# nh13/DWGSIM

Measured on AMD Instinct MI355X. Metric: M read-pairs/sec (2x150 bp PE), higher is better.
Workload: dtype u8

## Files before the change

### dwgsim_amd/csrc/dw_host.cpp

```cpp
#include <hip/hip_runtime.h>
#include <math.h>
#include <stdio.h>
#include <stdlib.h>
#include <string.h>
#include <limits.h>
#include <ctype.h>
#include <stdarg.h>
#include <stdint.h>
#include <sys/mman.h>
#include <mutex>
#include <thread>
#include <string>
#include <vector>
#include <algorithm>
#include <array>
#include <stddef.h>
#include <type_traits>
#include "../../include/dwgsim_hip.h"
#include "dw_kernels.hpp"
#include "dw_launch.hpp"
#include "dw_mutin.hpp"
#include "dw_mem.hpp"

using namespace dw;

namespace {

struct HostIns { std::vector<int32_t> pos; std::vector<uint32_t> len, off; std::vector<uint8_t> bases; };

struct Member {
    std::string name;
    int64_t l = 0, l_place = 0;
    uint32_t contig_index = 0;
    int32_t start = 0;
    int32_t reg_off = 0, n_reg = 0;
    uint32_t name_off = 0; int32_t name_fixed_len = 0;
    ResolvedContig rc;
};

struct GroupMem {
    DevMem d_ref, d_cells[2], d_view[2];
    DevMem d_ins_pos[2], d_ins_len[2], d_ins_off[2], d_ins_bases[2];
    DevMem d_names, d_reg, d_seg;
    std::vector<uint8_t> h_names; std::vector<int32_t> h_reg, h_seg;
    DevMem d_summ[2], d_summ2[2];
    DevMem d_refview, d_refsumm, d_refsumm2, d_dirty;
    DevEvent ev_walk, ev_walk0;
    DevMem d_hap_text[2], d_hap_rec, d_hap_pool;
    HostMem h_wc;
};

struct WalkCounters {
    uint64_t unused0[7];
    uint64_t n_cand;
    uint32_t max_del;
    struct { uint32_t entries, bases; } ins[2];
    uint32_t unused1;
    uint32_t slot_over;
    uint32_t n_cand_true;
    uint64_t mut_debug[2];
    uint64_t n_listed;
    uint64_t unused2;
};
static_assert(std::is_standard_layout<WalkCounters>::value && sizeof(WalkCounters) == 16 * 8, "the walk's counter block is 16 u64 words");
static_assert(offsetof(WalkCounters, n_cand) == 7 * 8 && offsetof(WalkCounters, max_del) == 8 * 8 && offsetof(WalkCounters, ins) == 8 * 8 + 4 && offsetof(WalkCounters, slot_over) == 8 * 8 + 6 * 4 &&
              offsetof(WalkCounters, n_cand_true) == 8 * 8 + 7 * 4 && offsetof(WalkCounters, mut_debug) == 12 * 8 && offsetof(WalkCounters, n_listed) == 14 * 8, "every counter at the word the kernels were given before the block had a type");
struct WcSpan { size_t off, bytes; };
#define WC_SPAN(first, last) WcSpan{offsetof(WalkCounters, first), offsetof(WalkCounters, last) + sizeof(WalkCounters::last) - offsetof(WalkCounters, first)}
constexpr WcSpan WC_RANDOM = WC_SPAN(n_cand, n_cand_true), WC_FILE = WC_SPAN(mut_debug, mut_debug), WC_LISTED = WC_SPAN(n_listed, n_listed);

struct Group {
    bool alive = false, mutated = false, walk_pending = false;
    int first_handle = -1;
    std::vector<Member> m;
    int64_t total = 0;
    GroupMem mem;
    uint32_t n_ins[2] = {0, 0}, n_ins_bases[2] = {0, 0};
    int fixed_max = 0;
    uint32_t n_cand = 0;
    bool dirty_any = false, dirty_all = false;
    int walk_attempt = 0; uint32_t walk_cap = 0; size_t walk_cap_bases = 0; bool walk_reset = false;
    uint32_t n_patch = 0, n_patch_ev = 0;
    bool list_valid = false; std::vector<int32_t> pos; std::vector<uint32_t> cells; HostIns ins[2];
    struct HapText { bool valid = false; int width = 0; uint64_t bytes = 0; std::vector<uint64_t> off, len; std::vector<int64_t> bases; } hap_text[2];
};

struct HandleRef { int group = -1, k = 0; };

constexpr int N_COUNTERS = 32;

struct Counters {
    DevMem d; HostMem h;
    uint64_t *dev() const { return d.get<uint64_t>(); }
    uint64_t *host() const { return h.get<uint64_t>(); }
};

struct Slot {
    Counters counters;
    hipEvent_t ev_k0 = nullptr, ev_k1 = nullptr, ev_end = nullptr, ev_done = nullptr, ev_fetched = nullptr;
    bool pending = false, empty = true, fetch_in_flight = false;
    int group = -1;
    uint64_t n_pairs = 0, out_bytes[3] = {0, 0, 0}, gz_bytes[3] = {0, 0, 0};
    DevMem gz_out[3], gz_status, segs;
    HostMem h_segs;
    std::vector<dwgsim_hip_range_t> ranges;
    DevMem d_rerun_chain;
    int cap_mult = 1;
};

}

struct dwgsim_hip_ctx {
    dwgsim_hip_params_t prm;
    std::string read_prefix;
    std::vector<uint8_t> flow;
    DevMem d_flow;
    int device = 0;
    hipStream_t stream = nullptr;
    hipStream_t copy_stream = nullptr;
    hipStream_t walk_stream = nullptr;
    hipStream_t count_stream = nullptr;
    std::string err;
    double e_by[2] = {0, 0};
    DevMem d_thr[2];
    DevMem d_thr32[2]; int e_full = 0;
    DevMem d_qbase[2]; int32_t qb_words = 1;
    DevMem d_rand_fixed; int32_t rand_fixed_len = 0;
    std::vector<Group> groups;
    std::vector<GroupMem> pool;
    std::vector<HandleRef> handles;
    DevMem meta, fail_summ, block_rand, status_all, out[DWGSIM_HIP_SLOTS][3], split_state, split_hand, split_agg, split_pre, split_chunk;
    DevMem w_slots, w_slot_aux;
    int site_slots = -1; int64_t site_slot_cap = -1;
    DevMem scratch_mask, scratch_cnt, scratch_status, w_cand, w_ev, w_flags, w_lo, w_sufmin, w_bound, w_ppos, w_pcells, up_ascii, l_pos, l_cells, place_segs, place_rand, place_list, place_aux;
    HostMem h_up; hipEvent_t ev_up = nullptr; bool up_in_flight = false;
    HostMem h_place_segs, h_range_rand;
    std::vector<int32_t> h_ppos; std::vector<uint16_t> h_pcells; std::vector<Event> h_pev;
    bool seq_justify = false, dense_view = false;
    MutInput mutin; bool has_mutin = false;
    Regions regions; bool has_regions = false;
    DevMem flow_scratch, flow_free;
    Counters counters;
    DevMem d_wcounters;
    Counters pcounters;
    Slot slot[DWGSIM_HIP_SLOTS];
    DevMem d_chain;
    int chain_contig = -1; uint64_t chain_next_ii = 0;
    bool has_carry_override = false; uint64_t carry_override = 0;
    int flow_cap_forced = 0;
    int flow_cap_mult = 1;
    int ion_lds = -1;
    int n_cu = 0; int flow_slots = 0;
    int64_t walk_cap = -1; bool phases = false; int writer = -1, force_threads = 0; int64_t place_cap = -1; uint64_t place_open = 0; double walk_us = 0, count_us = 0; int split = -1;
    int64_t sim_form = 0;
    int64_t walk_form = 0;
    hipEvent_t ev_cnt0 = nullptr, ev_cnt1 = nullptr;
    bool gzip_on = false; DevMem d_crc_table, d_crc_shift;
    HostMem h_stage;
    hipStream_t hap_stream = nullptr;
    DevEvent hap_ev[6]; double hap_len_us = 0, hap_write_us = 0, hap_copy_us = 0; bool hap_yardstick = false;
    int hap_cur[2] = {-1, -1};
    std::string txt, vcf;
};

namespace {

#define HIPC(ctx, call) do { hipError_t e_ = (call); if (e_ != hipSuccess) { char b_[512]; snprintf(b_, sizeof b_, "HIP error %s at %s:%d (%s)", hipGetErrorString(e_), __FILE__, __LINE__, #call); (ctx)->err = b_; return DWGSIM_HIP_ERR_DEVICE; } } while (0)

hipError_t dev_malloc(dwgsim_hip_ctx *c, void **p, size_t bytes)
{
    hipError_t e = DevKind::alloc(p, bytes);
    if (e == hipSuccess || c->pool.empty()) return e;
    (void)hipGetLastError();
    hipStreamSynchronize(c->walk_stream);
    c->pool.clear();
    return DevKind::alloc(p, bytes);
}

hipError_t reserve(dwgsim_hip_ctx *c, DevMem &b, size_t need, size_t want)
{
    return b.reserve(need, want, [c](void **p, size_t n) { return dev_malloc(c, p, n); });
}

int ensure(dwgsim_hip_ctx *c, DevMem &b, size_t bytes)
{
    HIPC(c, reserve(c, b, bytes, bytes + bytes / 8 + 4096));
    return 0;
}

int upload(dwgsim_hip_ctx *c, DevMem &b, const void *src, size_t n)
{
    HIPC(c, reserve(c, b, n, n));
    const hipError_t e = hipMemcpy(b.get(), src, n, hipMemcpyHostToDevice);
    if (e != hipSuccess) b.reset();
    HIPC(c, e);
    return 0;
}

template <class T> int upload_table(dwgsim_hip_ctx_t *c, DevMem &d, const std::vector<T> &h, size_t slack)
{
    HIPC(c, reserve(c, d, sizeof(T) * h.size(), sizeof(T) * (h.size() + slack)));
    HIPC(c, hipMemcpyAsync(d.get(), h.data(), sizeof(T) * h.size(), hipMemcpyHostToDevice, c->walk_stream));
    return 0;
}

uint8_t nt4(int ch)
{
    switch (ch) { case 'A': case 'a': return 0; case 'C': case 'c': return 1; case 'G': case 'g': return 2; case 'T': case 't': return 3; case '-': return 5; default: return 4; }
}

void lazy_quality_params(double sigma, float *k, float *eps, float *lmin, int32_t *near1_zero)
{
    const double two_ln2 = 2.0 * log(2.0);
    double lm = 0.98 * (0.45 / sigma) * (0.45 / sigma) / two_ln2;
    if (!(lm < 0x1p-4)) lm = 0x1p-4;
    *near1_zero = lm >= 0x1p-10 ? 1 : 0;
    if (lm < 0x1p-10) lm = 0x1p-10;
    *lmin = (float)lm;
    lm = (double)*lmin * (1.0 - 0x1p-20);
    *k = (float)(sqrt(two_ln2) * sigma);
    *eps = (float)(1.5 * sigma * (3.4e-7 / sqrt(lm) + 7.2e-6) + 0x1p-18);
}

WalkParams walk_params(const dwgsim_hip_ctx *c)
{
    WalkParams w; w.mut_rate = c->prm.mut_rate; w.indel_frac = c->prm.indel_frac; w.indel_extend = c->prm.indel_extend;
    w.indel_min = c->prm.indel_min; w.is_hap = c->prm.is_hap; w.seed = (uint32_t)c->prm.seed;
    w.mut_thr = !(c->prm.mut_rate > 0) ? 0 : c->prm.mut_rate >= 1.0 ? 0x100000000ull : (uint64_t)ceil(c->prm.mut_rate * 4294967296.0);
    flow_gap_params(w.mut_thr, &w.gap_r, &w.gap_s);
    w.lg = reinterpret_cast<const uint32_t *>(c->d_flow.get() + 64);
    return w;
}

size_t padded_cells(const Group &g) { return (size_t)g.total + CELL_PAD; }

size_t view_bytes(size_t padded) { return padded / 2; }
size_t summ_bytes(size_t padded) { return sizeof(uint16_t) * (padded / SUMM_CELLS); }
size_t summ2_bytes(size_t padded) { return sizeof(uint16_t) * (padded / SUMM2_CELLS); }
uint32_t dirty_words(size_t padded) { return (uint32_t)((padded + 32 * SUMM_CELLS - 1) / (32 * SUMM_CELLS)); }
size_t dirty_bytes(size_t padded) { return sizeof(uint32_t) * ((size_t)dirty_words(padded) + 2); }

enum : unsigned { R_CELLS = 1, R_VIEW = 2, R_SUMM = 4, R_SUMM2 = 8, R_ALL = 15 };
int restore_pristine(dwgsim_hip_ctx *c, const Group &g, int h, unsigned what, hipStream_t st)
{
    const GroupMem &M = g.mem;
    const size_t padded = padded_cells(g);
    if (what & R_CELLS) HIPC(c, hipMemcpyAsync(M.d_cells[h].get(), M.d_ref.get(), padded, hipMemcpyDeviceToDevice, st));
    if (what & R_VIEW) HIPC(c, hipMemcpyAsync(M.d_view[h].get(), M.d_refview.get(), view_bytes(padded), hipMemcpyDeviceToDevice, st));
    if (what & R_SUMM) HIPC(c, hipMemcpyAsync(M.d_summ[h].get(), M.d_refsumm.get(), summ_bytes(padded), hipMemcpyDeviceToDevice, st));
    if (what & R_SUMM2) HIPC(c, hipMemcpyAsync(M.d_summ2[h].get(), M.d_refsumm2.get(), summ2_bytes(padded), hipMemcpyDeviceToDevice, st));
    return 0;
}

int clear_dirty(dwgsim_hip_ctx *c, const Group &g, hipStream_t st)
{
    HIPC(c, hipMemsetAsync(g.mem.d_dirty.get(), 0, dirty_bytes(padded_cells(g)), st));
    return 0;
}

hipError_t wc_fill(dwgsim_hip_ctx *c, WcSpan s, int byte, hipStream_t st) { return hipMemsetAsync(c->d_wcounters.get() + s.off, byte, s.bytes, st); }
hipError_t wc_fetch(dwgsim_hip_ctx *c, const GroupMem &M, WcSpan s, hipStream_t st) { return hipMemcpyAsync(M.h_wc.get() + s.off, c->d_wcounters.get() + s.off, s.bytes, hipMemcpyDeviceToHost, st); }

struct InsTable { void *dev, *host; size_t bytes; };
std::array<InsTable, 4> ins_tables(const GroupMem &M, int h, HostIns &t)
{
    return {{{M.d_ins_pos[h].get(), t.pos.data(), sizeof(int32_t) * t.pos.size()}, {M.d_ins_len[h].get(), t.len.data(), sizeof(uint32_t) * t.len.size()},
             {M.d_ins_off[h].get(), t.off.data(), sizeof(uint32_t) * t.off.size()}, {M.d_ins_bases[h].get(), t.bases.data(), t.bases.size()}}};
}

SegTab seg_tab(const Group &g)
{
    const int n = (int)g.m.size();
    const int32_t *seg = g.mem.d_seg.get<int32_t>();
    SegTab t; t.start = seg; t.len = seg + (n + 1); t.cindex = reinterpret_cast<const uint32_t *>(seg + (2 * n + 1)); t.n = n;
    return t;
}

void fill_haps(const Group &g, HapDev (&hap)[2])
{
    const GroupMem &M = g.mem;
    for (int h = 0; h < 2; ++h) {
        hap[h].cells = M.d_cells[h].get(); hap[h].view = M.d_view[h].get(); hap[h].ins_pos = M.d_ins_pos[h].get<int32_t>(); hap[h].ins_len = M.d_ins_len[h].get<uint32_t>();
        hap[h].ins_off = M.d_ins_off[h].get<uint32_t>(); hap[h].ins_bases = M.d_ins_bases[h].get(); hap[h].n_ins = g.n_ins[h]; hap[h].pos_off = 0;
    }
}

ContigDev group_dev(const Group &g)
{
    ContigDev d;
    fill_haps(g, d.hap);
    d.ref = g.mem.d_ref.get(); d.l = g.total; d.seg = seg_tab(g);
    d.tot4 = nullptr; d.cap_bases[0] = d.cap_bases[1] = 0;
    return d;
}

size_t ins_bases_cap(const Group &g, int h) { const size_t cap = g.mem.d_ins_bases[h].cap(); return cap ? cap - 16 : 0; }

Group *get_group(dwgsim_hip_ctx_t *c, int contig, int *k = nullptr)
{
    if (!c) return nullptr;
    if (contig < 0 || (size_t)contig >= c->handles.size() || c->handles[(size_t)contig].group < 0) { c->err = "unknown contig handle"; return nullptr; }
    const HandleRef r = c->handles[(size_t)contig];
    Group &g = c->groups[(size_t)r.group];
    if (!g.alive) { c->err = "unknown contig handle"; return nullptr; }
    if (k) *k = r.k;
    return &g;
// ... 1155 lines not shown
    if (bytes) *bytes = T.len[(size_t)km];
    if (bases) *bases = T.bases[(size_t)km];
    return DWGSIM_HIP_OK;
}

int dwgsim_hip_haplotype_fetch(dwgsim_hip_ctx_t *c, int hap, uint64_t offset, void *host_dst, size_t n)
{
    if (!c) return DWGSIM_HIP_ERR_ARG;
    if (hap < 0 || hap > 1 || (!host_dst && n)) { c->err = "bad haplotype_fetch arguments"; return DWGSIM_HIP_ERR_ARG; }
    const int gid = c->hap_cur[hap];
    if (gid < 0 || !c->groups[(size_t)gid].alive || !c->groups[(size_t)gid].hap_text[hap].valid) { c->err = "haplotype_fetch: dwgsim_hip_haplotype_fasta must run first"; return DWGSIM_HIP_ERR_STATE; }
    const Group &g = c->groups[(size_t)gid];
    const uint64_t total = g.hap_text[hap].bytes;
    if (offset > total || (uint64_t)n > total - offset) { c->err = "haplotype_fetch: past the end of the text"; return DWGSIM_HIP_ERR_ARG; }
    if (n == 0) return DWGSIM_HIP_OK;
    HIPC(c, hipSetDevice(c->device));
    if (!c->hap_stream) HIPC(c, hipStreamCreate(&c->hap_stream));
    const uint8_t *src = g.mem.d_hap_text[hap].get<uint8_t>() + offset;
    if (is_page_locked(host_dst)) {
        HIPC(c, hipMemcpyAsync(host_dst, src, n, hipMemcpyDeviceToHost, c->hap_stream));
        HIPC(c, hipStreamSynchronize(c->hap_stream));
        return DWGSIM_HIP_OK;
    }
    const size_t CH = (size_t)16 << 20;
    HIPC(c, c->h_stage.reserve(2 * CH, 2 * CH));
    uint8_t *stage[2] = {c->h_stage.get<uint8_t>(), c->h_stage.get<uint8_t>() + CH};
    size_t done = 0; int b = 0;
    size_t cur = n < CH ? n : CH;
    HIPC(c, hipMemcpyAsync(stage[0], src, cur, hipMemcpyDeviceToHost, c->hap_stream));
    while (done < n) {
        HIPC(c, hipStreamSynchronize(c->hap_stream));
        const size_t next_off = done + cur, next = next_off < n ? ((n - next_off) < CH ? (n - next_off) : CH) : 0;
        if (next) HIPC(c, hipMemcpyAsync(stage[b ^ 1], src + next_off, next, hipMemcpyDeviceToHost, c->hap_stream));
        memcpy((uint8_t *)host_dst + done, stage[b], cur);
        done += cur; cur = next; b ^= 1;
    }
    return DWGSIM_HIP_OK;
}

namespace {
struct Launch { SimForm f; SimArgs a; Group *g = nullptr; std::vector<SimSeg> segs; uint64_t n_pairs = 0; uint32_t nblk = 0; int fixed_max = 0; };
struct SimPlan {
    size_t cap[3];
    int32_t lb_shift; bool too_many;
    size_t block_rand, status, meta, fail_summ, split_state, split_hand, split_agg, split_pre, split_chunk;
    bool scratch; int32_t flow_slots; size_t flow_scratch, flow_free;
    size_t segs, gz_chunks[3], gz_cap[3], gz_status;
};
struct ChainSet { uint64_t *words; int set_rand, set_carry; uint64_t carry; };
}

static int build_ranges(dwgsim_hip_ctx_t *c, const dwgsim_hip_range_t *r, int n, uint64_t ppb, Launch &L)
{
    if (!r || n < 1) { c->err = "bad range arguments"; return DWGSIM_HIP_ERR_ARG; }
    Group *g = nullptr;
    uint64_t pairs = 0, blocks = 0; int fmax = 0;
    std::vector<SimSeg> &segs = L.segs;
    segs.clear();
    for (int q = 0; q < n; ++q) {
        int k = 0;
        Group *gq = get_group(c, r[q].contig, &k);
        if (!gq) return DWGSIM_HIP_ERR_ARG;
        if (g && gq != g) { c->err = "the ranges of one call must belong to contigs that were added together (dwgsim_hip_add_contigs)"; return DWGSIM_HIP_ERR_ARG; }
        g = gq;
        if (r[q].n_pairs == 0) continue;
        const Member &m = g->m[(size_t)k];
        if (c->has_regions && m.n_reg == 0 && c->prm.rand_read < 1.0) { c->err = "dwgsim-hip: this contig has no target region (-x): the reference's placement loop would not terminate\n"; return DWGSIM_HIP_ERR_ARG; }
        SimSeg s; memset(&s, 0, sizeof s);
        s.first_block = (uint32_t)blocks; s.contig_index = m.contig_index; s.start = m.start; s.l = (int32_t)m.l;
        s.first_ii = r[q].first_ii; s.n_pairs = r[q].n_pairs; s.pair_off = pairs; s.l_place = m.l_place;
        s.reg_off = m.reg_off; s.n_reg = m.n_reg; s.name_off = m.name_off; s.name_fixed_len = m.name_fixed_len;
        s.contig_start = r[q].first_ii == 0 ? 1u : 0u;
        segs.push_back(s);
        pairs += r[q].n_pairs; blocks += (r[q].n_pairs + ppb - 1) / ppb;
        if (m.name_fixed_len > fmax) fmax = m.name_fixed_len;
        if (blocks > 0x7fffffffull) { c->err = "too many pairs in one call"; return DWGSIM_HIP_ERR_ARG; }
    }
    if (!g->mutated || g->walk_pending) { c->err = "mutate_contig must run first"; return DWGSIM_HIP_ERR_STATE; }
    L.g = g; L.n_pairs = pairs; L.nblk = (uint32_t)blocks; L.fixed_max = fmax;
    return DWGSIM_HIP_OK;
}

static int sim_form(dwgsim_hip_ctx_t *c, SimForm &f)
{
    const dwgsim_hip_params_t &p = c->prm;
    const size_t qb = (size_t)c->qb_words;
    const int lmax = p.length[0] > p.length[1] ? p.length[0] : p.length[1];
    f = SimForm();
    f.lpp = p.length[1] > 0 ? 2 : 1;
    f.out = (p.reads_output_type != 2 ? 1 : 0) | (p.reads_output_type != 1 ? 2 : 0);
    f.dt = p.data_type;
    f.nthr = SIM_THREADS;
    f.cap = lmax; f.lds_words = (lmax + 7) / 8;
    bool fifo = true;
    if (p.data_type == 0) {
        const int cap_fifo = 5, cap_reg = (p.reads_output_type == 0) ? 4 : 5;
        const int b_fifo = sim_blocks_per_cu(sim_lds_bytes((size_t)f.lds_words, SIM_THREADS, qb, true), cap_fifo), b_reg = sim_blocks_per_cu(sim_lds_bytes((size_t)f.lds_words, SIM_THREADS, qb, false), cap_reg);
        if (b_fifo < b_reg && !(p.reads_output_type == 0 && b_fifo >= 3)) fifo = false;
        if (c->writer >= 0) fifo = c->writer != 0;
    }
    const size_t need = sim_lds_bytes((size_t)f.lds_words, SIM_THREADS, qb, fifo);
    if (p.data_type != 2 && (need > SIM_LDS_BUDGET || ((sim_blocks_per_cu(need, 8) < 2 || c->force_threads == SIM_THREADS_LONG) && c->force_threads != SIM_THREADS))) {
        f.nthr = SIM_THREADS_LONG; fifo = true;
        if (sim_lds_bytes(0, SIM_THREADS_LONG, qb, true) > SIM_LDS_BUDGET) {
            char b[160]; snprintf(b, sizeof b, "dwgsim-hip: reads longer than %d bases are not supported for -c 0 / -c 1\n", (int)((SIM_LDS_BUDGET - SIM_THREADS_LONG * SIM_FIFO_BYTES) / 2 - 16));
            c->err = b; return DWGSIM_HIP_ERR_UNSUP;
        }
    }
    if (p.data_type == 2) {
        f.cap = std::max(flow_base_capacity(c), lmax) * c->flow_cap_mult;
        f.lds_words = (f.cap + 15) / 16; f.cap = 16 * f.lds_words;
        f.stack_words = std::min(FLOW_STACK_WORDS * c->flow_cap_mult, FLOW_STACK_WORDS_MAX);
        const size_t per_lane = (size_t)(f.lds_words + f.stack_words);
        const size_t need256 = sim_lds_bytes(per_lane, SIM_THREADS, qb, true), need64 = sim_lds_bytes(per_lane, ION_THREADS_SMALL, qb, true);
        int mode = c->ion_lds;
        if (mode < 0) mode = (need256 <= SIM_LDS_BUDGET && sim_blocks_per_cu(need256, 8) >= 2) ? 1 : (need64 <= SIM_LDS_BUDGET && sim_blocks_per_cu(need64, 32) >= 4) ? 2 : 0;
        if ((mode == 1 && need256 > SIM_LDS_BUDGET) || (mode == 2 && need64 > SIM_LDS_BUDGET)) mode = 0;
        f.dt = mode != 0 ? 3 : 2; f.nthr = mode == 2 ? ION_THREADS_SMALL : SIM_THREADS;
    }
    const bool split_wins = lmax <= 50;
    f.split = (p.data_type == 0 && f.nthr == SIM_THREADS && (c->split < 0 ? split_wins : c->split != 0)) ? 1 : 0;
    if (f.dt == 3 && f.nthr == SIM_THREADS && f.cap < 32768 && c->split != 0) f.split = 1;
    if (f.split && c->writer < 0) fifo = true;
    const size_t stage = f.dt == 3 ? (size_t)(f.lds_words + f.stack_words) : f.dt == 2 ? (size_t)f.stack_words : f.nthr != SIM_THREADS ? 0 : (size_t)f.lds_words;
    if (f.split) { f.wr = fifo ? 2 : 0; f.lds = sim_lds_bytes(stage, (size_t)f.nthr, 0, false); f.lds_b = sim_lds_bytes(0, (size_t)f.nthr, qb, fifo, SIM_FIFO_BYTES_WIDE); }
    else { f.wr = fifo ? 1 : 0; f.lds = sim_lds_bytes(stage, (size_t)f.nthr, qb, fifo); }
    return 0;
}

static void fill_sim_args(const dwgsim_hip_ctx_t *c, const Group &g, const SimForm &f, SimArgs &a)
{
    const dwgsim_hip_params_t &p = c->prm;
    memset(&a, 0, sizeof a);
    a.p.std_dev = p.std_dev; a.p.mut_freq = p.mut_freq; a.p.rand_read = p.rand_read; a.p.quality_std = p.quality_std;
    a.p.dist = p.dist; a.p.is_inner = p.is_inner; a.p.len[0] = p.length[0]; a.p.len[1] = p.length[1]; a.p.max_n = p.max_n;
    a.p.strandedness = p.strandedness; a.p.read_one_strand = p.read_one_strand; a.p.amplicons = p.amplicons;
    a.p.fixed_quality = p.fixed_quality; a.p.data_type = p.data_type;
    a.p.has_bfast = p.reads_output_type != 1; a.p.has_bwa = p.reads_output_type != 2;
    a.p.seed = (uint32_t)p.seed;
    lazy_quality_params(p.quality_std, &a.p.q_k, &a.p.q_eps, &a.p.q_lmin, &a.p.q_near1);
    fill_haps(g, a.hap);
    a.chain = c->d_chain.get<uint64_t>();
    a.have_regions = c->has_regions ? 1 : 0; a.reg = g.mem.d_reg.get<int32_t>();
    for (int j = 0; j < 2; ++j) { a.e_thr[j] = c->d_thr[j].get<uint64_t>(); a.e_thr32[j] = c->d_thr32[j].get<uint32_t>(); a.qbase[j] = c->d_qbase[j].get<uint32_t>() ? c->d_qbase[j].get<uint32_t>() : c->d_qbase[0].get<uint32_t>(); }
    a.qb_words = c->qb_words;
    a.e_full = c->e_full;
    a.names = g.mem.d_names.get();
    a.summ[0] = g.mem.d_summ[0].get<uint16_t>(); a.summ[1] = g.mem.d_summ[1].get<uint16_t>(); a.summ2[0] = g.mem.d_summ2[0].get<uint16_t>(); a.summ2[1] = g.mem.d_summ2[1].get<uint16_t>();
    a.place_fast = (!c->has_regions && !p.amplicons && p.std_dev * 12.1 + 2.0 < 1e9) ? 1 : 0;
    a.place_k = a.place_fast ? (int32_t)ceil(p.std_dev * 12.1) + 2 : 0;
    a.rand_fixed = c->d_rand_fixed.get(); a.rand_fixed_len = c->rand_fixed_len;
    a.sim_threads = f.nthr; a.fifo = f.wr != 0; a.split = f.split; a.ion_lds = f.dt == 3;
    a.cap = f.cap; a.lds_words = f.lds_words; a.flow_stack_words = f.stack_words;
    a.flow = c->d_flow.get(); a.flow_len = (int32_t)c->flow.size();
    for (int j = 0; j < 2; ++j) {
        const int n = c->prm.length[j];
        uint64_t tmax = 0, tmin = ~0ull;
        for (int i = 0; i < n; ++i) {
            const double ei = c->prm.e_start[j] + c->e_by[j] * i;
            const uint64_t t = !(ei > 0) ? 0 : ei >= 1.0 ? 0x100000000ull : (uint64_t)ceil(ei * 4294967296.0);
            tmax = std::max(tmax, t); tmin = std::min(tmin, t);
        }
        a.err_thr_max[j] = n > 0 ? tmax : 0; a.err_ramp[j] = (n > 0 && tmin != tmax) ? 1 : 0;
        flow_gap_params(a.err_thr_max[j], &a.err_gap_r[j], &a.err_gap_s[j]);
    }
    for (int j = 0; j < 2; ++j) {
        const double e0 = c->prm.e_start[j];
        flow_gap_params(!(e0 > 0) ? 0 : e0 >= 1.0 ? 0x100000000ull : (uint64_t)ceil(e0 * 4294967296.0), &a.flow_gap_r[j], &a.flow_gap_s[j]);
    }
}

static int sim_resolve(dwgsim_hip_ctx_t *c, const dwgsim_hip_range_t *r, int n, Launch &L)
{
    if (!r || n < 1) { c->err = "bad range arguments"; return DWGSIM_HIP_ERR_ARG; }
    if (!get_group(c, r[0].contig)) return DWGSIM_HIP_ERR_ARG;
    if (const int rc = sim_form(c, L.f)) return rc;
    if (const int rc = build_ranges(c, r, n, (uint64_t)(L.f.nthr / L.f.lpp), L)) return rc;
    fill_sim_args(c, *L.g, L.f, L.a);
    return DWGSIM_HIP_OK;
}

int dwgsim_hip_count_random_ranges(dwgsim_hip_ctx_t *c, const dwgsim_hip_range_t *r, int n, uint64_t *n_random, uint64_t *per_range)
{
    if (!c) return DWGSIM_HIP_ERR_ARG;
    if (n_random) *n_random = 0;
    if (per_range) for (int q = 0; q < n; ++q) per_range[q] = 0;
    Launch L;
    if (const int rc = build_ranges(c, r, n, PLACE_PAIRS, L)) return rc;
    const uint64_t n_pairs = L.n_pairs; const uint32_t n_blocks = L.nblk;
    if (n_pairs == 0) return DWGSIM_HIP_OK;
    Group &g = *L.g;
    HIPC(c, hipSetDevice(c->device));
    hipStream_t st = c->count_stream;
    if (g.walk_pending) { if (const int rc = dwgsim_hip_mutate_wait(c, g.first_handle)) return rc; }
    if (g.mem.ev_walk.get() && g.mutated) HIPC(c, hipStreamWaitEvent(st, g.mem.ev_walk.get(), 0));
    if (const int rc = sim_form(c, L.f)) return rc;
    SimArgs &a = L.a; fill_sim_args(c, g, L.f, a);
    const size_t ns = L.segs.size();
    if (ensure(c, c->place_rand, sizeof(uint32_t) * ((size_t)n_blocks + 1)) || ensure(c, c->place_segs, sizeof(SimSeg) * ns) ||
        ensure(c, c->place_aux, PLACE_LISTS * 16 * sizeof(uint32_t) + sizeof(uint64_t) * ns)) return DWGSIM_HIP_ERR_DEVICE;
    if (sizeof(SimSeg) * ns > c->h_place_segs.cap() || sizeof(uint64_t) * ns > c->h_range_rand.cap()) HIPC(c, hipStreamSynchronize(st));
    HIPC(c, c->h_place_segs.reserve(sizeof(SimSeg) * ns, sizeof(SimSeg) * (ns + 64))); HIPC(c, c->h_range_rand.reserve(sizeof(uint64_t) * ns, sizeof(uint64_t) * (ns + 64)));
    const uint64_t *h_range_rand = c->h_range_rand.get<uint64_t>();
    memcpy(c->h_place_segs.get(), L.segs.data(), sizeof(SimSeg) * ns);
    HIPC(c, hipMemcpyAsync(c->place_segs.get(), c->h_place_segs.get(), sizeof(SimSeg) * ns, hipMemcpyHostToDevice, st));
    a.segs = c->place_segs.get<SimSeg>(); a.n_seg = (int32_t)ns; a.n_blocks = n_blocks; a.n_pairs = n_pairs;
    a.block_rand = c->place_rand.get<uint32_t>(); a.counters = c->pcounters.dev();
    const uint64_t waves = (uint64_t)n_blocks * (PLACE_PAIRS / 64);
    const uint32_t cap_full = (uint32_t)((waves + PLACE_LISTS - 1) / PLACE_LISTS) * 64u;
    uint32_t cap = (uint32_t)std::min<uint64_t>(cap_full, 1024 + n_pairs / PLACE_LISTS / 8);
    if (c->place_cap >= 0 && (uint64_t)c->place_cap < cap) cap = (uint32_t)c->place_cap;
    for (int attempt = 0;; ++attempt) {
        if (ensure(c, c->place_list, sizeof(uint32_t) * (size_t)cap * PLACE_LISTS)) return DWGSIM_HIP_ERR_DEVICE;
        a.place_list = c->place_list.get<uint32_t>(); a.place_list_cap = cap;
        a.place_list_n = c->place_aux.get<uint32_t>(); a.range_rand = reinterpret_cast<uint64_t *>(c->place_aux.get<uint8_t>() + PLACE_LISTS * 16 * sizeof(uint32_t));
        HIPC(c, hipMemsetAsync(c->pcounters.dev(), 0, N_COUNTERS * sizeof(uint64_t), st));
        HIPC(c, hipMemsetAsync(c->place_aux.get(), 0, PLACE_LISTS * 16 * sizeof(uint32_t) + sizeof(uint64_t) * ns, st));
        HIPC(c, hipEventRecord(c->ev_cnt0, st));
        launch_place(st, a);
        HIPC(c, hipEventRecord(c->ev_cnt1, st));
        HIPC(c, hipGetLastError());
        HIPC(c, hipMemcpyAsync(c->pcounters.host(), c->pcounters.dev(), N_COUNTERS * sizeof(uint64_t), hipMemcpyDeviceToHost, st));
        HIPC(c, hipMemcpyAsync(c->h_range_rand.get(), a.range_rand, sizeof(uint64_t) * ns, hipMemcpyDeviceToHost, st));
        HIPC(c, hipStreamSynchronize(st));
        { float ms = 0; if (hipEventElapsedTime(&ms, c->ev_cnt0, c->ev_cnt1) == hipSuccess) c->count_us += 1e3 * ms; else (void)hipGetLastError(); }
        if (!(c->pcounters.host()[2] & 16) || attempt > 0) break;
        cap = cap_full;
    }
    if (c->pcounters.host()[2] & 16) { c->err = "count_random: the list of undecided pairs overflowed twice"; return DWGSIM_HIP_ERR_FAILED; }
    if (c->pcounters.host()[2]) { char b[128]; snprintf(b, sizeof b, "\r[dwgsim_core] failed to generate a read after %d trials\n", MAX_ATTEMPTS + 1); c->err = b; return DWGSIM_HIP_ERR_FAILED; }
    c->place_open = c->pcounters.host()[5];
    uint64_t total = 0;
    for (int q = 0, si = 0; q < n; ++q) if (r[q].n_pairs) { total += h_range_rand[si]; if (per_range) per_range[q] = h_range_rand[si]; ++si; }
    if (n_random) *n_random = total;
    return DWGSIM_HIP_OK;
}

int dwgsim_hip_count_random(dwgsim_hip_ctx_t *c, int contig, uint64_t first_ii, uint64_t n_pairs, uint64_t *n_random)
{
    dwgsim_hip_range_t r; memset(&r, 0, sizeof r); r.contig = contig; r.first_ii = first_ii; r.n_pairs = n_pairs;
    return dwgsim_hip_count_random_ranges(c, &r, 1, n_random, nullptr);
}

int dwgsim_hip_set_fail_carry(dwgsim_hip_ctx_t *c, uint64_t carry)
{
    if (!c) return DWGSIM_HIP_ERR_ARG;
    c->carry_override = carry; c->has_carry_override = true;
    return DWGSIM_HIP_OK;
}

static SimPlan sim_plan(const dwgsim_hip_ctx_t *c, const Launch &L)
{
    const dwgsim_hip_params_t &p = c->prm; const SimForm &f = L.f;
    const uint64_t n_pairs = L.n_pairs; const size_t nblk = L.nblk;
    SimPlan P{};
    const int fixed_max = std::max(L.fixed_max, c->rand_fixed_len);
    for (int j = 0; j < 2; ++j) if (p.length[j] > 0) P.cap[j] = (size_t)n_pairs * (size_t)(1 + fixed_max + 120 + 3 + 2 * (p.data_type == 2 ? f.cap : p.length[j]) + 4);
    int bw_bytes = 0, bw_pairs = 0;
    while (bw_bytes < 63 && (((uint64_t)P.cap[0] | 1ull) >> bw_bytes)) ++bw_bytes;
    while (bw_pairs < 63 && (n_pairs >> bw_pairs)) ++bw_pairs;
    P.lb_shift = bw_bytes; P.too_many = p.data_type != 2 && bw_bytes + bw_pairs > 62;
    P.cap[2] = P.cap[0] + P.cap[1];
    if (!L.a.p.has_bwa) P.cap[0] = P.cap[1] = 0;
    if (!L.a.p.has_bfast) P.cap[2] = 0;
    P.block_rand = sizeof(uint32_t) * nblk;
    if (!f.split) P.status = 4 * sizeof(uint64_t) * nblk;
    else { P.split_state = sizeof(uint32_t) * (size_t)f.lds_words * SIM_THREADS * nblk; P.split_hand = 16 * (size_t)SIM_THREADS * nblk; P.split_agg = 16 * nblk; P.split_pre = 32 * nblk; P.split_chunk = 32 * (nblk / 1024 + 1); }
    P.meta = sizeof(uint32_t) * ((size_t)n_pairs + 8);
    P.fail_summ = ((size_t)((n_pairs + 256ull * 64 - 1) / (256ull * 64)) * 4 + 2) * sizeof(uint64_t);
    P.scratch = f.dt == 2 || (f.dt < 2 && f.nthr == SIM_THREADS_LONG);
    if (P.scratch) {
        const int cu_per_xcd = (c->n_cu >= 64 && c->n_cu % 8 == 0) ? c->n_cu / 8 : c->n_cu;
        const bool ion = p.data_type == 2;
        const int per_cu = sim_blocks_per_cu(f.lds, ion ? 8 : 32);
        P.flow_slots = c->flow_slots > 0 ? c->flow_slots : cu_per_xcd * per_cu;
        if ((uint64_t)P.flow_slots > (uint64_t)nblk) P.flow_slots = (int32_t)nblk;
        if (ion) {
            const size_t slot_bytes = (size_t)flow_words_per_lane(f.lds_words) * (size_t)SIM_THREADS * sizeof(uint32_t);
            const size_t fit = std::max<size_t>(1, ((size_t)4 << 30) / (slot_bytes * 8));
            if ((size_t)P.flow_slots > fit) P.flow_slots = (int32_t)fit;
        }
        const size_t words = (ion ? (size_t)flow_words_per_lane(f.lds_words) * (size_t)SIM_THREADS : (size_t)f.lds_words * (size_t)SIM_THREADS_LONG) * (size_t)P.flow_slots * 8;
        P.flow_scratch = words * sizeof(uint32_t); P.flow_free = sizeof(uint64_t) * (256 + 8 * nblk);
    }
    P.segs = sizeof(SimSeg) * L.segs.size();
    if (c->gzip_on) {
        size_t chunks = 0;
        for (int t = 0; t < 3; ++t) { P.gz_chunks[t] = (size_t)gz_chunks(P.cap[t]); chunks += P.gz_chunks[t]; if (P.cap[t]) P.gz_cap[t] = (size_t)gz_capacity(P.cap[t]); }
        P.gz_status = sizeof(uint64_t) * (chunks ? chunks : 1);
    }
    return P;
}

static int sim_reserve(dwgsim_hip_ctx_t *c, int slot, const SimPlan &P)
{
    Slot &sl = c->slot[slot]; DevMem *out = c->out[slot];
    if (sl.fetch_in_flight) { HIPC(c, hipStreamWaitEvent(c->stream, sl.ev_fetched, 0)); bool grows = false; for (int t = 0; t < 3; ++t) if (P.cap[t] + 64 > out[t].cap()) grows = true; if (grows) HIPC(c, hipEventSynchronize(sl.ev_fetched)); sl.fetch_in_flight = false; }
    for (int t = 0; t < 3; ++t) if (ensure(c, out[t], P.cap[t] + 64)) return DWGSIM_HIP_ERR_DEVICE;
    if (ensure(c, c->block_rand, P.block_rand) || ensure(c, c->status_all, P.status) ||
        ensure(c, c->split_state, P.split_state) || ensure(c, c->split_hand, P.split_hand) || ensure(c, c->split_agg, P.split_agg) || ensure(c, c->split_pre, P.split_pre) || ensure(c, c->split_chunk, P.split_chunk) ||
        ensure(c, c->meta, P.meta) || ensure(c, c->fail_summ, P.fail_summ) || ensure(c, c->flow_scratch, P.flow_scratch) || ensure(c, c->flow_free, P.flow_free) || ensure(c, sl.segs, P.segs)) return DWGSIM_HIP_ERR_DEVICE;
    HIPC(c, sl.h_segs.reserve(P.segs, P.segs + 64 * sizeof(SimSeg)));
    for (int t = 0; t < 3; ++t) if (P.gz_cap[t] && ensure(c, sl.gz_out[t], P.gz_cap[t] + 64)) return DWGSIM_HIP_ERR_DEVICE;
    return ensure(c, sl.gz_status, P.gz_status);
}

// ... 156 lines not shown
    auto touch = [p](size_t from, size_t upto) { for (size_t o = from; o < upto; o += 4096) ((volatile uint8_t *)p)[o] = 0; };
    const int nt = len >= ((size_t)64 << 20) ? 4 : 1;
    if (nt == 1) touch(0, len);
    else {
        std::vector<std::thread> th; const size_t per = (len / H + (size_t)nt - 1) / (size_t)nt * H;
        for (int k = 0; k < nt; ++k) { const size_t a = std::min(len, (size_t)k * per), b = std::min(len, a + per); if (b > a) th.emplace_back(touch, a, b); }
        for (auto &t : th) t.join();
    }
    if (hipHostRegister(p, len, hipHostRegisterDefault) != hipSuccess) { (void)hipGetLastError(); munmap(p, len); return nullptr; }
    { std::lock_guard<std::mutex> lk(g_host_m); g_host.push_back(HostRegion{p, len}); }
    return p;
}
void dwgsim_hip_host_free(void *p)
{
    if (!p) return;
    HostRegion r{nullptr, 0};
    {
        std::lock_guard<std::mutex> lk(g_host_m);
        for (size_t i = 0; i < g_host.size(); ++i) if (g_host[i].base == (uint8_t *)p) { r = g_host[i]; g_host.erase(g_host.begin() + (long)i); break; }
    }
    if (!r.base) return;
    (void)hipHostUnregister(r.base);
    munmap(r.base, r.len);
}

static int fetch_async(dwgsim_hip_ctx_t *c, int slot, int stream, void *host_dst, size_t cap, bool gz)
{
    if (!c || slot < 0 || slot >= DWGSIM_HIP_SLOTS || stream < 0 || stream > 2 || (!host_dst && cap)) { if (c) c->err = "bad fetch arguments"; return DWGSIM_HIP_ERR_ARG; }
    Slot &sl = c->slot[slot];
    if (sl.pending) { c->err = "fetch: wait for the batch first (its sizes are not known yet)"; return DWGSIM_HIP_ERR_STATE; }
    HIPC(c, hipSetDevice(c->device));
    const size_t n = (size_t)(gz ? sl.gz_bytes[stream] : sl.out_bytes[stream]);
    if (n > cap) { c->err = "fetch: destination too small"; return DWGSIM_HIP_ERR_ARG; }
    if (n == 0) return DWGSIM_HIP_OK;
    HIPC(c, hipMemcpyAsync(host_dst, gz ? sl.gz_out[stream].get() : c->out[slot][stream].get(), n, hipMemcpyDeviceToHost, c->copy_stream));
    HIPC(c, hipEventRecord(sl.ev_fetched, c->copy_stream));
    sl.fetch_in_flight = true;
    return DWGSIM_HIP_OK;
}
int dwgsim_hip_fetch_async(dwgsim_hip_ctx_t *c, int slot, int stream, void *host_dst, size_t cap) { return fetch_async(c, slot, stream, host_dst, cap, false); }

int dwgsim_hip_set_gzip(dwgsim_hip_ctx_t *c, int on)
{
    if (!c) return DWGSIM_HIP_ERR_ARG;
    HIPC(c, hipSetDevice(c->device));
    if (on && !c->d_crc_shift) {
        std::vector<uint32_t> tab(4 * 256), sh(16 * 1024);
        gz_host_tables(tab.data(), sh.data());
        if (upload(c, c->d_crc_table, tab.data(), tab.size() * 4) || upload(c, c->d_crc_shift, sh.data(), sh.size() * 4)) return DWGSIM_HIP_ERR_DEVICE;
    }
    c->gzip_on = on != 0;
    return DWGSIM_HIP_OK;
}

int dwgsim_hip_fetch_gz_async(dwgsim_hip_ctx_t *c, int slot, int stream, void *host_dst, size_t cap) { return fetch_async(c, slot, stream, host_dst, cap, true); }

int dwgsim_hip_fetch_wait(dwgsim_hip_ctx_t *c, int slot)
{
    if (!c || slot < 0 || slot >= DWGSIM_HIP_SLOTS) { if (c) c->err = "bad slot"; return DWGSIM_HIP_ERR_ARG; }
    Slot &sl = c->slot[slot];
    if (!sl.fetch_in_flight) return DWGSIM_HIP_OK;
    HIPC(c, hipSetDevice(c->device));
    HIPC(c, hipEventSynchronize(sl.ev_fetched));
    sl.fetch_in_flight = false;
    return DWGSIM_HIP_OK;
}

int dwgsim_hip_fetch(dwgsim_hip_ctx_t *c, int slot, int stream, void *host_dst, size_t cap)
{
    if (!c || slot < 0 || slot >= DWGSIM_HIP_SLOTS || stream < 0 || stream > 2 || (!host_dst && cap)) return DWGSIM_HIP_ERR_ARG;
    HIPC(c, hipSetDevice(c->device));
    Slot &sl = c->slot[slot];
    if (sl.pending) { c->err = "fetch: wait for the batch first (its sizes are not known yet)"; return DWGSIM_HIP_ERR_STATE; }
    const size_t n = (size_t)sl.out_bytes[stream];
    if (n > cap) { c->err = "fetch: destination too small"; return DWGSIM_HIP_ERR_ARG; }
    if (n == 0) return DWGSIM_HIP_OK;
    if (is_page_locked(host_dst)) {
        HIPC(c, hipMemcpyAsync(host_dst, c->out[slot][stream].get(), n, hipMemcpyDeviceToHost, c->copy_stream));
        HIPC(c, hipStreamSynchronize(c->copy_stream));
        return DWGSIM_HIP_OK;
    }
    const size_t CH = (size_t)16 << 20;
    HIPC(c, c->h_stage.reserve(2 * CH, 2 * CH));
    const uint8_t *src = c->out[slot][stream].get<uint8_t>();
    uint8_t *stage[2] = {c->h_stage.get<uint8_t>(), c->h_stage.get<uint8_t>() + CH};
    size_t done = 0; int b = 0;
    size_t cur = n < CH ? n : CH;
    HIPC(c, hipMemcpyAsync(stage[0], src, cur, hipMemcpyDeviceToHost, c->copy_stream));
    while (done < n) {
        HIPC(c, hipStreamSynchronize(c->copy_stream));
        const size_t next_off = done + cur, next = next_off < n ? ((n - next_off) < CH ? (n - next_off) : CH) : 0;
        if (next) HIPC(c, hipMemcpyAsync(stage[b ^ 1], src + next_off, next, hipMemcpyDeviceToHost, c->copy_stream));
        memcpy((uint8_t *)host_dst + done, stage[b], cur);
        done += cur; cur = next; b ^= 1;
    }
    return DWGSIM_HIP_OK;
}

int dwgsim_hip_debug_count_byte(dwgsim_hip_ctx_t *c, int slot, int stream, int byte, uint64_t *count)
{
    if (!c || slot < 0 || slot >= DWGSIM_HIP_SLOTS || stream < 0 || stream > 2 || !count) return DWGSIM_HIP_ERR_ARG;
    HIPC(c, hipSetDevice(c->device));
    Slot &sl = c->slot[slot];
    if (sl.pending) { c->err = "count_byte: wait for the batch first"; return DWGSIM_HIP_ERR_STATE; }
    HIPC(c, hipMemsetAsync(&c->counters.dev()[15], 0, sizeof(uint64_t), c->stream));
    if (sl.out_bytes[stream]) launch_count_byte(c->stream, c->out[slot][stream].get<uint8_t>(), sl.out_bytes[stream], (uint32_t)(byte & 0xff), &c->counters.dev()[15]);
    HIPC(c, hipMemcpyAsync(&c->counters.host()[15], &c->counters.dev()[15], sizeof(uint64_t), hipMemcpyDeviceToHost, c->stream));
    HIPC(c, hipStreamSynchronize(c->stream));
    *count = c->counters.host()[15];
    return DWGSIM_HIP_OK;
}

int dwgsim_hip_debug_gzip(dwgsim_hip_ctx_t *c, const void *text, size_t n, void *out, size_t cap, size_t *out_n)
{
    if (!c || (!text && n) || !out_n) return DWGSIM_HIP_ERR_ARG;
    HIPC(c, hipSetDevice(c->device));
    if (const int rc = dwgsim_hip_set_gzip(c, c->gzip_on ? 1 : 0); rc < 0) return rc;
    if (!c->d_crc_shift) { const bool was = c->gzip_on; if (const int rc = dwgsim_hip_set_gzip(c, 1); rc < 0) return rc; c->gzip_on = was; }
    *out_n = 0;
    if (n == 0) return DWGSIM_HIP_OK;
    const size_t gcap = (size_t)gz_capacity(n), nch = (size_t)gz_chunks(n);
    DevMem text_m, out_m, aux_m;
    if (reserve(c, text_m, n + 64, n + 64) != hipSuccess || reserve(c, out_m, gcap + 64, gcap + 64) != hipSuccess || reserve(c, aux_m, sizeof(uint64_t) * (4 + nch), sizeof(uint64_t) * (4 + nch)) != hipSuccess) { c->err = "out of device memory"; return DWGSIM_HIP_ERR_DEVICE; }
    uint8_t *d_text = text_m.get(), *d_out = out_m.get(); uint64_t *d_aux = aux_m.get<uint64_t>();
    const uint64_t n64 = n;
    bool ok = hipMemcpyAsync(d_text, text, n, hipMemcpyHostToDevice, c->stream) == hipSuccess && hipMemsetAsync(d_aux, 0, sizeof(uint64_t) * (4 + nch), c->stream) == hipSuccess &&
              hipMemcpyAsync(d_aux, &n64, sizeof n64, hipMemcpyHostToDevice, c->stream) == hipSuccess;
    if (ok) {
        launch_gzip(c->stream, d_text, &d_aux[0], n, d_out, gcap, &d_aux[4], &d_aux[1], &d_aux[2], &d_aux[3], c->d_crc_table.get<uint32_t>(), c->d_crc_shift.get<uint32_t>());
        uint64_t res[4] = {0, 0, 0, 0};
        ok = hipGetLastError() == hipSuccess && hipMemcpyAsync(res, d_aux, sizeof res, hipMemcpyDeviceToHost, c->stream) == hipSuccess && hipStreamSynchronize(c->stream) == hipSuccess;
        if (ok && (res[3] & 8)) { c->err = "dwgsim-hip: the gzip output buffer is too small for this text\n"; return DWGSIM_HIP_ERR_FAILED; }
        if (ok && res[2] > cap) { c->err = "debug_gzip: destination too small"; return DWGSIM_HIP_ERR_ARG; }
        if (ok) { ok = hipMemcpy(out, d_out, (size_t)res[2], hipMemcpyDeviceToHost) == hipSuccess; *out_n = (size_t)res[2]; }
    }
    if (!ok) { c->err = "debug_gzip: device error"; return DWGSIM_HIP_ERR_DEVICE; }
    return DWGSIM_HIP_OK;
}

int dwgsim_hip_debug_option(dwgsim_hip_ctx_t *c, const char *key, int64_t value)
{
    if (!c || !key) return DWGSIM_HIP_ERR_ARG;
    if (!strcmp(key, "justify_seq")) c->seq_justify = value != 0;
    else if (!strcmp(key, "dense_view")) c->dense_view = value != 0;
    else if (!strcmp(key, "walk_cap")) c->walk_cap = value;
    else if (!strcmp(key, "site_slots")) c->site_slots = (int)value;
    else if (!strcmp(key, "site_slot_cap")) c->site_slot_cap = value;
    else if (!strcmp(key, "phases")) c->phases = value != 0;
    else if (!strcmp(key, "writer")) c->writer = (int)value;
    else if (!strcmp(key, "sim_threads")) c->force_threads = (int)value;
    else if (!strcmp(key, "walk_seg_min")) walk_debug_seg_min((uint32_t)value);
    else if (!strcmp(key, "place_cap")) c->place_cap = value;
    else if (!strcmp(key, "split")) c->split = (int)value;
    else if (!strcmp(key, "flow_slots")) c->flow_slots = (int)value;
    else if (!strcmp(key, "ion_lds")) c->ion_lds = (int)value;
    else if (!strcmp(key, "flow_cap")) c->flow_cap_forced = (int)value;
    else if (!strcmp(key, "hap_yardstick")) c->hap_yardstick = value != 0;
    else { c->err = "unknown debug option"; return DWGSIM_HIP_ERR_ARG; }
    return DWGSIM_HIP_OK;
}

int dwgsim_hip_debug_get(dwgsim_hip_ctx_t *c, const char *key, int64_t *value)
{
    if (!c || !key || !value) return DWGSIM_HIP_ERR_ARG;
    if (!strcmp(key, "place_open")) *value = (int64_t)c->place_open;
    else if (!strcmp(key, "flow_cap_mult")) *value = (int64_t)c->flow_cap_mult;
    else if (!strcmp(key, "walk_us")) *value = (int64_t)c->walk_us;
    else if (!strcmp(key, "count_us")) *value = (int64_t)c->count_us;
    else if (!strcmp(key, "sim_form")) *value = c->sim_form;
    else if (!strcmp(key, "hap_len_us")) *value = (int64_t)c->hap_len_us;
    else if (!strcmp(key, "hap_write_us")) *value = (int64_t)c->hap_write_us;
    else if (!strcmp(key, "hap_copy_us")) *value = (int64_t)c->hap_copy_us;
    else if (!strcmp(key, "walk_form")) *value = c->walk_form;
    else { c->err = "unknown debug value"; return DWGSIM_HIP_ERR_ARG; }
    return DWGSIM_HIP_OK;
}

int dwgsim_hip_debug_sim_instances(int64_t *out, int cap)
{
    return sim_instances(out, cap);
}

}
```

### dwgsim_amd/csrc/dw_kernels.hpp

```cpp
#pragma once
#include <stdint.h>

namespace dw {

constexpr int PAIRS_PER_BLOCK = 128;
constexpr int PLACE_PAIRS = 256;
constexpr int PLACE_LISTS = 64;
#ifndef DW_SIM_THREADS
#define DW_SIM_THREADS 256
#endif
constexpr int SIM_THREADS = DW_SIM_THREADS;
constexpr int FLOW_STACK_WORDS = 4;
constexpr uint32_t FLOW_NEVER = 0xFFFFFFFFu;
constexpr int FLOW_LG_ENTRIES = 257;
constexpr int FLOW_CAP_MAX = 1 << 20;
constexpr int FLOW_STACK_WORDS_MAX = 32;
#ifndef DW_ION_THREADS_SMALL
#define DW_ION_THREADS_SMALL 128
#endif
constexpr int ION_THREADS_SMALL = DW_ION_THREADS_SMALL;
constexpr int SIM_THREADS_LONG = 64;
constexpr int SIM_FIFO_BYTES = 40;
constexpr int SIM_FIFO_BYTES_WIDE = 72;
inline size_t sim_lds_bytes(size_t words_per_lane, size_t lanes, size_t qb_words, bool fifo, size_t fifo_bytes = SIM_FIFO_BYTES) { return ((words_per_lane * lanes + 2 * qb_words + 3) & ~(size_t)3) * 4 + (fifo ? lanes * fifo_bytes : 0); }
// ... 15 lines not shown

struct Event {
    int32_t  pos;
    uint8_t  type;
    uint8_t  hap;
    uint8_t  base;
    uint8_t  live;
    uint32_t len;
    uint32_t seg;
};

struct SegTab { const int32_t *start; const int32_t *len; const uint32_t *cindex; int32_t n; };

struct HapDev {
    uint8_t *cells;
    const uint8_t *view;
    int32_t *ins_pos;
    uint32_t *ins_len;
    uint32_t *ins_off;
    uint8_t *ins_bases;
    uint32_t n_ins;
    int32_t pos_off;
};

struct ContigDev {
    HapDev hap[2];
    const uint8_t *ref;
    int64_t l;
    SegTab seg;
    const uint32_t *tot4;
    uint32_t cap_bases[2];
};

struct HapRec { uint64_t rec_off; uint32_t hdr_off, hdr_len, base0, n_bases; uint32_t pad_; };
constexpr int HAP_WINDOW = 8192;

struct Count { const uint64_t *dev; uint32_t host; };

struct WalkParams {
    double mut_rate, indel_frac, indel_extend;
    uint64_t mut_thr;
    uint64_t gap_r; int32_t gap_s;
    const uint32_t *lg;
    int32_t indel_min, is_hap;
    uint32_t seed;
};

struct SimParams {
    double std_dev, mut_freq, rand_read, quality_std;
    int32_t dist, is_inner, len[2], max_n, strandedness, read_one_strand, amplicons, fixed_quality, data_type;
    int32_t has_bwa, has_bfast;
    uint32_t seed;
    float q_k, q_eps, q_lmin; int32_t q_near1;
};

inline uint64_t flow_ilog2_fixed(uint64_t y, int fb)
{
    const int p = 63 - __builtin_clzll(y);
    uint64_t m = y << (63 - p), frac = 0;
    for (int k = 0; k < fb; ++k) {
        const unsigned __int128 sq = (unsigned __int128)m * m;
        if ((uint64_t)(sq >> 127)) { m = (uint64_t)(sq >> 64); frac = (frac << 1) | 1u; }
        else { m = (uint64_t)(sq >> 63); frac <<= 1; }
    }
    return ((uint64_t)p << fb) | frac;
}
inline void flow_log2_table(uint32_t *lg)
{
    for (int i = 0; i < 256; ++i) lg[i] = (uint32_t)flow_ilog2_fixed(256u + (uint64_t)i, 32);
    lg[256] = 0xFFFFFFFFu;
}
inline void flow_gap_params(uint64_t thr, uint64_t *R, int32_t *s)
{
    *R = 0; *s = 0;
    if (thr == 0 || thr >= 0x100000000ull) return;
    const uint64_t Lq = (32ull << 56) - flow_ilog2_fixed(0x100000000ull - thr, 56);
    const int sh = __builtin_clzll(Lq);
    const unsigned __int128 q = ((unsigned __int128)1 << 127) / (Lq << sh);
    if ((uint64_t)(q >> 64)) { *R = 1ull << 63; *s = 62 - sh; }
    else { *R = (uint64_t)q; *s = 63 - sh; }
}

struct CalibArgs {
    uint32_t seed; int32_t end, len; uint64_t n_reads, first_read, chunk_reads;
    uint64_t thr;
    uint64_t gap_r; int32_t gap_s;
    const uint8_t *flow; int32_t flow_len, lds_words, stack_words;
    uint32_t *scratch;
    uint64_t *counters;
};

constexpr int SUMM_CELLS = 64;
constexpr int SUMM2_CELLS = 1024;

inline constexpr int flow_words_per_lane(int lds_words) { return lds_words | 1; }

struct SimSeg {
    uint32_t first_block;
    uint32_t contig_index;
    int32_t  start, l;
    uint64_t first_ii, n_pairs;
    uint64_t pair_off;
    int64_t  l_place;
    int32_t  reg_off, n_reg;
    uint32_t name_off; int32_t name_fixed_len;
    uint32_t contig_start;
    uint32_t pad_;
};

struct SimArgs {
    SimParams p;
    HapDev hap[2];
    const SimSeg *segs; int32_t n_seg; uint32_t n_blocks;
    uint64_t n_pairs;
    const uint64_t *chain;
    const int32_t *reg; int32_t have_regions;
    const uint64_t *e_thr[2];
    const uint16_t *summ[2];
    const uint16_t *summ2[2];
    int32_t place_fast, place_k;
    uint32_t *place_list, *place_list_n; uint32_t place_list_cap;
    uint64_t *range_rand;
    const uint32_t *e_thr32[2];
    int32_t e_full;
    const uint32_t *qbase[2];
    int32_t qb_words;
    const uint8_t *names;
    const uint8_t *rand_fixed; int32_t rand_fixed_len;
    uint32_t *meta;
    uint32_t *block_rand;
    uint64_t *counters;
    uint64_t *status[4];
    uint8_t *out[3];
    int32_t lds_words;
    int32_t cap;
    int32_t ion_lds;
    int32_t flow_stack_words;
    int32_t fifo;
    int32_t sim_threads;
    int32_t flow_len;
    int32_t split;
    uint32_t *split_state;
    uint32_t *split_hand;
    uint32_t *split_agg;
    uint64_t *split_pre;
    uint64_t *split_chunk;
    uint32_t *flow_scratch;
    uint64_t *flow_free;
    int32_t flow_slots;
    int32_t lb_shift;
    const uint8_t *flow;
    uint64_t flow_gap_r[2]; int32_t flow_gap_s[2];
    uint64_t err_thr_max[2], err_gap_r[2]; int32_t err_gap_s[2], err_ramp[2];
};

}
```

### dwgsim_amd/csrc/dw_read.hpp

```cpp
#pragma once
#include "dw_device.hpp"
#include <dw_probe.hpp>

namespace dw {

struct ReadRes { int32_t ext_coor, n_sub, n_indel, num_n, n_ins; };

DW_DEV uint64_t reverse_nibbles(uint64_t x)
{
    x = __builtin_bswap64(x);
    return ((x >> 4) & 0x0F0F0F0F0F0F0F0Full) | ((x & 0x0F0F0F0F0F0F0F0Full) << 4);
}
DW_DEV uint32_t reverse_nibbles32(uint32_t x)
{
    x = __builtin_bswap32(x);
    return ((x >> 4) & 0x0F0F0F0Fu) | ((x & 0x0F0F0F0Fu) << 4);
}
struct __attribute__((packed, aligned(4))) ViewQuad { uint32_t a, b, c, d; };
constexpr int WIN_CHUNKS = 6, WIN_WORDS = 4 * WIN_CHUNKS - 1;
struct NoSink { DW_DEV void put(int, uint32_t, int) const {} };
struct WordSink { uint32_t *lds; int stride; DW_DEV void put(int kw, uint32_t codes, int) const { lds[kw * stride] = codes; } };
DW_DEV uint32_t nibbles_to_pairs(uint32_t v)
{
    v = (v | (v >> 2)) & 0x0F0F0F0Fu; v = (v | (v >> 4)) & 0x00FF00FFu; return (v | (v >> 8)) & 0xFFFFu;
}
DW_DEV uint32_t pairs_to_nibbles(uint32_t v)
{
    v = (v | (v << 8)) & 0x00FF00FFu; v = (v | (v << 4)) & 0x0F0F0F0Fu; return (v | (v << 2)) & 0x33333333u;
}
DW_DEV uint32_t reverse_pairs16(uint32_t v)
{
    v = __builtin_bitreverse32(v) >> 16;
    return ((v & 0x5555u) << 1) | ((v >> 1) & 0x5555u);
}
struct FlowSink {
    uint32_t *buf; int stride, h0; bool rev;
    DW_DEV void put(int kw, uint32_t codes, int) const
    {
        uint32_t p = nibbles_to_pairs(codes & 0x33333333u & ~(((codes >> 2) & 0x11111111u) * 3u));
        if (rev) p = reverse_pairs16(p);
        const int h = rev ? h0 - kw : h0 + kw;
        reinterpret_cast<uint16_t *>(buf + (h >> 1) * stride)[h & 1] = (uint16_t)p;
    }
};
template <class Sink>
DW_DEV ReadRes gen_read(const HapDev &h, int64_t l, int64_t start, int step, int s, int strand, const Sink &sink)
{
    ReadRes r{-10, 0, 0, 0, 0};
    const bool fwd = step > 0;
    const int32_t li = (int32_t)l;
    int k = 0;
    int32_t i = (start < -0x7fffffffll || start > 0x7fffffffll) ? -1 : (int32_t)start;
    uint32_t accw = 0; int na = 0;
    auto emit = [&](uint32_t v) {
        if (strand) v = v < 4 ? 3 - v : 4;
        r.num_n += (v == 4);
        accw |= (v > 4u ? 4u : v) << (4 * na); ++k;
        if (++na == 8) { sink.put((k >> 3) - 1, accw, 8); accw = 0; na = 0; }
    };
    const uint32_t *const vw = reinterpret_cast<const uint32_t *>(h.view);
    while (k < s) {
        const int words_left = (s - k + 7) >> 3, nw = words_left < WIN_WORDS ? words_left : WIN_WORDS;
        const int cells = (s - k) < 8 * nw ? (s - k) : 8 * nw;
        const int nch = (nw + 4) >> 2;
        const int32_t b0 = i >> 3, eb = i >> 3;
        const bool win = i >= 0 && i < li && (fwd ? i <= li - cells : (i - cells + 1 >= 0 && eb - 4 * nch + 1 >= 0));
        bool esc = !win;
        if (win) {
            uint32_t X[4 * WIN_CHUNKS];
#pragma unroll
            for (int c = 0; c < WIN_CHUNKS; ++c) {
                ViewQuad q{0, 0, 0, 0};
                if (c < nch) q = *reinterpret_cast<const ViewQuad *>(vw + (fwd ? b0 + 4 * c : eb - 4 * c - 3));
                X[4 * c] = fwd ? q.a : q.d; X[4 * c + 1] = fwd ? q.b : q.c; X[4 * c + 2] = fwd ? q.c : q.b; X[4 * c + 3] = fwd ? q.d : q.a;
            }
            const bool d1 = !fwd && ((uint32_t)i & 7u) != 7u;
            const uint32_t sh = 4u * ((fwd ? (uint32_t)i : (uint32_t)i + 1u) & 7u);
            bool go = true;
#pragma unroll
            for (int w = 0; w < WIN_WORDS; ++w) {
                if (!(go && w < nw)) continue;
                const int want = s - k < 8 ? s - k : 8;
                const uint32_t lo = d1 ? X[w + 1] : X[w], hi = d1 ? X[w] : X[w + 1];
                uint32_t x = __builtin_amdgcn_alignbit(hi, lo, sh);
                if (!fwd) x = reverse_nibbles32(x);
                if (want < 8) x &= (1u << (4 * want)) - 1u;
                const uint32_t n8 = x & 0x88888888u;
                if (n8 & ((x & 0x77777777u) + 0x77777777u)) { esc = true; go = false; }
                else {
                    if (r.ext_coor < 0) { r.ext_coor = i; if (strand) r.ext_coor -= s - 1; }
                    r.n_sub += __popc(x & 0x44444444u);
                    r.num_n += __popc(n8);
                    uint32_t codes = x & 0x33333333u;
                    if (strand) codes = (codes ^ 0x33333333u) & ~((n8 >> 3) * 3u);
                    if (want < 8) codes &= (1u << (4 * want)) - 1u;
                    codes |= n8 >> 1;
                    sink.put(k >> 3, codes, want);
                    k += want; i += fwd ? want : -want;
                }
            }
        }
        if (!esc) continue;
        const int32_t ck_base = (i < 0 || i >= li) ? 0 : fwd ? (i & ~3) : ((i | 3) - 15 < 0 ? 0 : (i | 3) - 15);
        const ViewQuad ckq = *reinterpret_cast<const ViewQuad *>(h.cells + ck_base);
        const uint32_t ck0 = ckq.a, ck1 = ckq.b, ck2 = ckq.c, ck3 = ckq.d;
        const uint8_t *const cellp = h.cells;
        auto cell_at = [=](int32_t q) -> uint32_t {
            const uint32_t o = (uint32_t)(q - ck_base);
            if (o >= 16u) return cellp[q];
            const uint32_t w01 = (o & 4u) ? ck1 : ck0, w23 = (o & 4u) ? ck3 : ck2;
            return (((o & 8u) ? w23 : w01) >> (8u * (o & 3u))) & 0xffu;
        };
        for (;;) {
            if (i < 0 || i >= li) { k = -1; break; }
            const uint32_t c = cell_at(i), mt = c & TMASK;
            if (r.ext_coor < 0) {
                if (mt != T_NONE && mt != T_SUB) { i += step; continue; }
                r.ext_coor = i;
                if (strand) r.ext_coor -= s - 1;
            }
            if (mt == T_DEL) { ++r.n_indel; if (strand) r.ext_coor--; }
            else if (mt == T_NONE || mt == T_SUB) { emit(c & 0xf); if (mt == T_SUB) ++r.n_sub; }
            else {
                ++r.n_indel; ++r.n_ins;
                const uint32_t idx = ins_find(h, i);
                uint32_t n = h.ins_len[idx];
                const uint8_t *P = h.ins_bases + h.ins_off[idx];
                if (!strand) {
                    if (k < s) emit(c & 0xf);
                    for (uint32_t t = 0; t < n && k < s; ++t) emit(P[t] & 3u);
                } else {
                    while (n > 0 && k < s) { r.ext_coor++; emit(P[n - 1] & 3u); --n; }
                    if (k < s) emit(c & 0xf);
                }
            }
            i += step;
            if (k >= s || na == 0) break;
        }
        if (k < 0) break;
    }
    if (k != s) { r.ext_coor = -10; return r; }
    if (na) sink.put(k >> 3, accw, na);
    return r;
}

struct PairDraw { bool is_rand; int32_t pos, d; int hap, strand0, strand1; };

struct SegCtx {
    int64_t l, l_place;
    int32_t start;
    const int32_t *reg_start, *reg_end; int32_t n_reg;
};
DW_DEV HapDev sel_hap(const SimArgs &a, const SegCtx &sc, int h)
{
    HapDev r;
    r.cells = (h ? a.hap[1].cells : a.hap[0].cells) + sc.start;
    r.view = (h ? a.hap[1].view : a.hap[0].view) + (sc.start >> 1);
    r.ins_pos = h ? a.hap[1].ins_pos : a.hap[0].ins_pos;
    r.ins_len = h ? a.hap[1].ins_len : a.hap[0].ins_len;
    r.ins_off = h ? a.hap[1].ins_off : a.hap[0].ins_off;
    r.ins_bases = h ? a.hap[1].ins_bases : a.hap[0].ins_bases;
    r.n_ins = h ? a.hap[1].n_ins : a.hap[0].n_ins;
    r.pos_off = sc.start;
    return r;
}
typedef const DW_CONST_AS SimSeg *SegPtr;
DW_DEV uint32_t seg_of_block(SegPtr segs, int32_t n_seg, uint32_t t)
{
    uint32_t lo = 0, hi = (uint32_t)n_seg;
    while (hi - lo > 1) { const uint32_t mid = (lo + hi) >> 1; if (segs[mid].first_block <= t) lo = mid; else hi = mid; }
    return lo;
}
DW_DEV SegCtx seg_ctx(const SimArgs &a, SegPtr sg)
{
    SegCtx sc; sc.l = sg->l; sc.l_place = sg->l_place; sc.start = sg->start;
    sc.reg_start = a.reg ? a.reg + sg->reg_off : nullptr; sc.reg_end = a.reg ? a.reg + sg->reg_off + sg->n_reg : nullptr; sc.n_reg = sg->n_reg;
    return sc;
}
DW_DEV int sel_len(const SimArgs &a, int j) { return j ? a.p.len[1] : a.p.len[0]; }

DW_DEV PairDraw draw_pair(const SimArgs &a, const SegCtx &sc, RngKey key, uint64_t ii, uint32_t att)
{
    PairDraw pd; pd.pos = 0; pd.d = 0; pd.hap = 0; pd.strand0 = pd.strand1 = 0;
    const U4 b0 = rng_block(key, D_PAIR, ii, att, 0, 0);
    pd.is_rand = !(a.p.rand_read < u_lo(b0));
    if (pd.is_rand) return pd;
    const int s0 = a.p.len[0], s1 = a.p.len[1];
    const int64_t l = sc.l_place, sl = sc.l;
    if (a.p.amplicons) { pd.pos = 0; pd.d = (int32_t)sl; }
    else {
        uint32_t t = 0; int32_t pos, d; bool continue_flag = false;
        do {
            if (s1 > 0 && probe::off(32)) d = a.p.dist;
            else if (s1 > 0) {
                double v1, v2, rsq; uint32_t r = 0;
                do {
                    const U4 b = rng_block(key, D_PLACE_NORM, ii, att, r, t);
                    v1 = 2.0 * u_lo(b) - 1.0; v2 = 2.0 * u_hi(b) - 1.0;
                    rsq = v1 * v1 + v2 * v2; ++r;
                } while (rsq >= 1.0 || rsq == 0.0);
                const double fac = rsq >= 0x1p-60 ? sqrt_mid(div_mid(-2.0 * det_log<true>(rsq), rsq)) : sqrt(-2.0 * det_log(rsq) / rsq);
                double ran = v2 * fac;
                ran = ran * a.p.std_dev + a.p.dist;
                d = (int32_t)(ran + 0.5);
                const int32_t min_dist = s0 + s1;
                if (d < min_dist) d = min_dist;
                if ((int64_t)d > l) d = (int32_t)l;
            } else d = 0;
            const int64_t range = l - d + 1;
            pos = (int32_t)((double)range * rng_slot(key, D_PLACE, ii, att, t));
            bool inside = true;
            if (a.have_regions) {
                for (int q = 0; q < sc.n_reg; ++q) {
                    const int32_t jl = sc.reg_end[q] - sc.reg_start[q];
                    if (pos < jl) { pos = sc.reg_start[q] + pos - 1; break; }
                    pos -= jl;
                }
                inside = false;
                int lo = 0, hi = sc.n_reg - 1;
                const uint32_t qs = (uint32_t)pos, qe = (uint32_t)(pos + d);
                while (lo <= hi) {
                    const int mid = lo + (hi - lo) / 2;
                    if (qs < (uint32_t)sc.reg_start[mid]) hi = mid - 1;
                    else if ((uint32_t)sc.reg_end[mid] < qe) lo = mid + 1;
                    else { inside = true; break; }
                }
            }
            ++t;
            if (t > (1u << 20) || ((t & 1023u) == 0 && (__hip_atomic_load(&a.counters[2], __ATOMIC_RELAXED, __HIP_MEMORY_SCOPE_AGENT) & 4ull))) { pd.hap = -1; break; }
            continue_flag = !inside;
        } while (continue_flag || pos < 0 || pos >= sl || (int64_t)pos + d - 1 >= sl
                 || (s1 > 0 && !a.p.is_inner && ((s0 > 0 && d <= s1) || (d <= s0 && s1 > 0))));
        pd.pos = pos; pd.d = d;
    }
    if (pd.hap < 0) { pd.hap = 0; pd.pos = 0; pd.d = 0; pd.is_rand = true; atomicOr((unsigned long long *)&a.counters[2], 4ull); return pd; }
    pd.hap = u_hi(b0) < a.p.mut_freq ? 0 : 1;
    switch (a.p.read_one_strand) {
    case 0: pd.strand0 = rng_slot(key, D_PAIR, ii, att, 2) < 0.5 ? 1 : 0; break;
    case 1: pd.strand0 = 0; break;
    default: pd.strand0 = 1; break;
    }
    switch (a.p.strandedness) {
    case 0: pd.strand1 = (a.p.data_type == 0) ? 1 - pd.strand0 : pd.strand0; break;
    case 1: pd.strand1 = pd.strand0; break;
    default: pd.strand1 = 1 - pd.strand0; break;
    }
    return pd;
}

DW_DEV void read_geom(const SimArgs &a, const SegCtx &sc, const PairDraw &pd, int j, int64_t *start, int *step)
{
    const int64_t pos = pd.pos, d = pd.d, s0 = a.p.len[0], s1 = a.p.len[1], sl = sc.l;
    const bool amp = a.p.amplicons != 0, inner = a.p.is_inner != 0;
    if (s1 > 0) {
        const int64_t far_outer = pos + d - 1;
        if (pd.strand0 == pd.strand1) {
            if (pd.strand0 == 0) {
                if (j == 0) { *start = amp ? sl - 1 : (inner ? pos + s1 + d - 1 : pos + d - s0); *step = 1; }
                else { *start = pos; *step = 1; }
            } else {
                if (j == 0) { *start = pos + s0 - 1; *step = -1; }
                else { *start = amp ? sl - 1 : (inner ? pos + s0 + d + s1 - 1 : far_outer); *step = -1; }
            }
        } else {
            if (pd.strand0 == 0) {
                if (j == 0) { *start = pos; *step = 1; }
                else { *start = amp ? sl - 1 : (inner ? pos + s0 + d + s1 - 1 : far_outer); *step = -1; }
            } else {
                if (j == 0) { *start = amp ? sl - 1 : (inner ? pos + s1 + d + s0 - 1 : far_outer); *step = -1; }
                else { *start = pos; *step = 1; }
            }
        }
    } else {
        if (pd.strand0 == 0) { *start = pos; *step = 1; }
        else if (amp) { *start = sl - 1; *step = -1; }
        else { *start = pos + s0 - 1; *step = -1; }
    }
}

struct FlowRng {
    uint32_t seed, contig, dom, att, evt, s, w0, w1, w2, w3; uint64_t ii;
    DW_DEV void open(uint32_t event) { evt = event; s = 0; }
    DW_DEV uint32_t next()
    {
        if ((s & 3) == 0) { const U4 b = rng_block(RngKey{seed, contig}, dom + D_FLOW_EV, ii, att, s >> 2, evt); w0 = b.x; w1 = b.y; w2 = b.z; w3 = b.w; }
        const uint32_t k = s & 3; ++s;
        const uint32_t lo = (k & 1) ? w1 : w0, hi = (k & 1) ? w3 : w2;
        return (k & 2) ? hi : lo;
    }
    DW_DEV int more_errors(uint64_t thr) { int n = 1; while ((uint64_t)next() < thr && n < (1 << 14)) ++n; return n; }
};
struct Buf2 {
    const uint32_t *base; int stride, nw;
    DW_DEV uint32_t word(int w) const { return w < nw ? base[w * stride] : 0u; }
    DW_DEV uint32_t get8(int p) const
// ... 175 lines not shown
    if (!failed && n1 > 0 && n1 < capb) {
        const int D = capb - n1, dw = D >> 4; const uint32_t sh = ((uint32_t)D & 15u) * 2u;
        uint32_t hi = buf[(capw - 1 - dw) * stride];
        for (int j = capw - 1; j >= dw; --j) {
            const uint32_t lo = j - dw - 1 >= 0 ? buf[(j - dw - 1) * stride] : 0u;
            buf[j * stride] = sh ? __builtin_amdgcn_alignbit(hi, lo, 32u - sh) : hi;
            hi = lo;
        }
    }

    const uint32_t dom2 = rg.dom + D_FLOW_PASS2;
    const int in2 = capb - n1;
    BitAppender<2> o2; o2.init(buf, stride);
    auto stk_get = [&](int k) -> uint32_t { return (stk[(k >> 1) * stride] >> ((k & 1) * 16)) & 0xffffu; };
    auto stk_set = [&](int k, uint32_t v) { const uint32_t sh = (uint32_t)(k & 1) * 16; uint32_t w = stk[(k >> 1) * stride]; stk[(k >> 1) * stride] = (w & ~(0xffffu << sh)) | (v << sh); };
    int t2 = 0, sp = 0;
    auto settle = [&](uint32_t x) {
        if (sp == 0) { o2.push(x); ++t2; }
        else if (o2.n >= in2 + t2) failed = true;
        else {
            const uint32_t top = stk_get(sp - 1);
            o2.push(top >> 14);
            if ((top & 0x3fffu) <= 1) --sp; else stk_set(sp - 1, top - 1);
        }
    };
    rg.dom = dom2;
    G.m = 0; G.next = FLOW_NEVER;
    G.draw(__ballot(!failed) != 0, key, dom2, rg.ii, rg.att, 0u, thr, T.lg, gap_R, gap_s);
    {
        bool done = failed, parked = false; uint32_t g = 0, x = 0;
        for (;;) {
            const bool act = !done && !parked;
            if (act && sp == 0 && t2 >= n1) done = true;
            const bool go = act && !done;
            if (__ballot(go)) {
                const uint32_t v = B.get16(in2 + t2);
                const int n = !go ? 0 : n1 - t2 < 16 ? n1 - t2 : 16;
                uint32_t rem = G.next - g;
                int m = 0; bool ok = true;
#pragma unroll
                for (int p = 0; p < 8; ++p) {
                    const uint32_t e = T.pair[(flow_i << 4) | ((v >> (4 * p)) & 15u)], kt = e >> 8;
                    ok = ok && 2 * p + 2 <= n && kt <= rem;
                    if (ok) { rem -= kt; flow_i = e & 63u; m += 2; }
                }
                if (m < n) {
                    const uint32_t i1 = (flow_i << 2) | ((v >> (2 * m)) & 3u), k = T.dist[i1];
                    if (k <= rem) { rem -= k; flow_i = T.next1[i1]; ++m; }
                }
                g = G.next - rem;
                o2.push_many(m < 16 ? v & ((1u << (2 * m)) - 1u) : v, m);
                t2 += m;
                if (m < n) { x = (v >> (2 * m)) & 3u; parked = true; }
            }
            const uint64_t pm = __ballot(parked);
            if (pm && (__popcll(pm) >= FLOW_EVENT_BATCH || __ballot(!done && !parked) == 0)) {
                if (parked) {
                    for (;;) {
                        uint32_t left = T.dist[(flow_i << 2) | x];
                        const uint32_t q = G.next - g, skip = q < left ? q : left;
                        { uint32_t f = flow_i + skip; if (f >= (uint32_t)F) f -= (uint32_t)F; flow_i = f; }
                        g += skip; left -= skip;
                        if (left == 0) {
                            settle(x);
                            if (failed) { done = true; break; }
                            if (sp == 0) break;
                            x = stk_get(sp - 1) >> 14;
                            continue;
                        }
                        E.resolve(key, dom2, rg.ii, rg.att, g, thr);
                        int n_err;
                        if (E.oc & 0x200u) { rg.open(g); n_err = rg.more_errors(thr); } else n_err = (int)(E.oc & 0xffu);
                        if ((int)flow_i != marked_flow) {
                            if (sp >= stack_runs || n_err >= (1 << 14)) { failed = true; done = true; break; }
                            stk_set(sp, ((uint32_t)T.flow[flow_i] << 14) | (uint32_t)n_err); ++sp; total += n_err;
                        }
                        flow_i = flow_i + 1u == (uint32_t)F ? 0u : flow_i + 1u;
                        ++g;
                        G.draw(true, key, dom2, rg.ii, rg.att, g, thr, T.lg, gap_R, gap_s);
                    }
                    parked = false;
                }
            }
            if (__ballot(!done) == 0) break;
        }
    }
    if (failed) return -1;
    o2.flush();
    *n_err_out += total;
    return o2.n;
}

struct __attribute__((packed, aligned(1))) Unal16 { uint64_t a, b; };
struct __attribute__((packed, aligned(1))) Unal8 { uint64_t v; };
struct __attribute__((packed, aligned(1))) Unal4 { uint32_t v; };
struct __attribute__((packed, aligned(1))) Unal2 { uint16_t v; };
struct Writer {
    uint8_t *p; uint64_t lo, hi; uint32_t n;
    DW_DEV void init(uint8_t *q) { p = q; lo = hi = 0; n = 0; }
    DW_DEV void init(uint8_t *, uint8_t *q) { init(q); }
    DW_DEV void emit()
    {
        if (probe::off(2)) probe::keep(lo, hi, p);
        else { Unal16 v; v.a = lo; v.b = hi; *reinterpret_cast<Unal16 *>(p) = v; }
        p += 16; lo = hi = 0; n = 0;
    }
    DW_DEV void put(uint32_t b)
    {
        if (probe::off(1)) return;
        if (probe::off(64)) { probe::keep(b); return; }
        const uint64_t v = (uint64_t)b << (8 * (n & 7));
        if (n < 8) lo |= v; else hi |= v;
        if (++n == 16) emit();
    }
    DW_DEV void putn(uint64_t v, uint32_t cnt)
    {
        if (probe::off(1)) return;
        if (probe::off(64)) { probe::keep(v, cnt); return; }
        const uint32_t sh = 8 * (n & 7);
        if (n < 8) { lo |= v << sh; if (sh) hi |= v >> (64 - sh); }
        else hi |= v << sh;
        const uint32_t total = n + cnt;
        if (total >= 16) {
            const uint32_t over = total - 16;
            const uint64_t carry = over ? v >> (8 * (cnt - over)) : 0;
            emit();
            lo = carry; n = over;
        } else n = total;
    }
    DW_DEV void put4(uint32_t w) { putn((uint64_t)w, 4); }
    DW_DEV void put_lead8(uint32_t lead, uint64_t v, uint32_t cnt)
    {
        if (cnt < 8) putn((uint64_t)lead | (v << 8), cnt + 1);
        else { putn((uint64_t)lead | (v << 8), 8); putn(v >> 56, 1); }
    }
    DW_DEV void put16(uint32_t a, uint32_t b, uint32_t c, uint32_t d)
    {
        if (probe::off(1)) return;
        if (probe::off(64)) { probe::keep(a, b, c, d); return; }
        const uint64_t x = (uint64_t)a | ((uint64_t)b << 32), y = (uint64_t)c | ((uint64_t)d << 32);
        if (n == 0) { lo = x; hi = y; emit(); }
        else { putn(x, 8); putn(y, 8); }
    }
    DW_DEV void flush()
    {
        if (probe::off(2)) { probe::keep(lo, hi, p, n); p += n; lo = hi = 0; n = 0; return; }
        if (n & 8) { Unal8 v; v.v = lo; *reinterpret_cast<Unal8 *>(p) = v; p += 8; lo = hi; }
        if (n & 4) { Unal4 v; v.v = (uint32_t)lo; *reinterpret_cast<Unal4 *>(p) = v; p += 4; lo >>= 32; }
        if (n & 2) { Unal2 v; v.v = (uint16_t)lo; *reinterpret_cast<Unal2 *>(p) = v; p += 2; lo >>= 16; }
        if (n & 1) { *p = (uint8_t)lo; p += 1; }
        lo = hi = 0; n = 0;
    }
};
template <uint32_t BURST>
DW_DEV void fifo_store_range(const uint8_t *f, uint8_t *dst, uint32_t from, uint32_t upto)
{
    auto ld8 = [&](uint32_t b) { return *reinterpret_cast<const uint64_t *>(f + b); };
    auto st16 = [&](uint32_t b) { *reinterpret_cast<uint4 *>(dst + b) = make_uint4((uint32_t)ld8(b), (uint32_t)(ld8(b) >> 32), (uint32_t)ld8(b + 8), (uint32_t)(ld8(b + 8) >> 32)); };
    uint32_t b = from;
    if ((b & 1u) && b + 1 <= upto) { dst[b] = f[b]; b += 1; }
    if ((b & 2u) && b + 2 <= upto) { *reinterpret_cast<uint16_t *>(dst + b) = *reinterpret_cast<const uint16_t *>(f + b); b += 2; }
    if ((b & 4u) && b + 4 <= upto) { *reinterpret_cast<uint32_t *>(dst + b) = *reinterpret_cast<const uint32_t *>(f + b); b += 4; }
    if ((b & 8u) && b + 8 <= upto) { *reinterpret_cast<uint64_t *>(dst + b) = ld8(b); b += 8; }
    if (b + 16 <= upto) { st16(b); b += 16; }
    if (BURST == 64u) { if (b + 16 <= upto) { st16(b); b += 16; } if (b + 16 <= upto) { st16(b); b += 16; } }
    if (b + 8 <= upto) { *reinterpret_cast<uint64_t *>(dst + b) = ld8(b); b += 8; }
    if (b + 4 <= upto) { *reinterpret_cast<uint32_t *>(dst + b) = *reinterpret_cast<const uint32_t *>(f + b); b += 4; }
    if (b + 2 <= upto) { *reinterpret_cast<uint16_t *>(dst + b) = *reinterpret_cast<const uint16_t *>(f + b); b += 2; }
    if (b + 1 <= upto) { dst[b] = f[b]; }
}
template <uint32_t BURST>
DW_DEV void fifo_store_range_unaligned(const uint8_t *f, uint8_t *dstb, uint32_t from, uint32_t upto)
{
    if (from >= upto) return;
    auto ld8u = [&](uint32_t b) { return reinterpret_cast<const Unal8 *>(f + b)->v; };
    uint32_t b = from; const uint32_t n = upto - from;
    if (BURST == 64u && (n & 64u)) { for (int q = 0; q < 4; ++q) { Unal16 v; v.a = ld8u(b); v.b = ld8u(b + 8); *reinterpret_cast<Unal16 *>(dstb + b) = v; b += 16; } }
    if (n & 32u) { for (int q = 0; q < 2; ++q) { Unal16 v; v.a = ld8u(b); v.b = ld8u(b + 8); *reinterpret_cast<Unal16 *>(dstb + b) = v; b += 16; } }
    if (n & 16u) { Unal16 v; v.a = ld8u(b); v.b = ld8u(b + 8); *reinterpret_cast<Unal16 *>(dstb + b) = v; b += 16; }
    if (n & 8u) { Unal8 v; v.v = ld8u(b); *reinterpret_cast<Unal8 *>(dstb + b) = v; b += 8; }
    if (n & 4u) { Unal4 v = *reinterpret_cast<const Unal4 *>(f + b); *reinterpret_cast<Unal4 *>(dstb + b) = v; b += 4; }
    if (n & 2u) { Unal2 v = *reinterpret_cast<const Unal2 *>(f + b); *reinterpret_cast<Unal2 *>(dstb + b) = v; b += 2; }
    if (n & 1u) { dstb[b] = f[b]; }
}
template <uint32_t BURST = 32u, bool DUAL = false>
struct FifoWriter {
    uint8_t *f, *dst; uint32_t wp, skip;
    uint8_t *dstb; uint32_t bdone;
    DW_DEV void init(uint8_t *fifo, uint8_t *rec) { const uint32_t h = (uint32_t)((uintptr_t)rec & (BURST - 1u)); f = fifo; dst = rec - h; wp = skip = h; }
    DW_DEV void init(uint8_t *fifo, uint8_t *rec, uint8_t *rec_b) { init(fifo, rec); dstb = rec_b - skip; bdone = skip; }
    DW_DEV uint64_t ld8(uint32_t b) const { return *reinterpret_cast<const uint64_t *>(f + b); }
    DW_DEV uint64_t ld8u(uint32_t b) const { return reinterpret_cast<const Unal8 *>(f + b)->v; }
    DW_DEV void st16(uint32_t b) const { *reinterpret_cast<uint4 *>(dst + b) = make_uint4((uint32_t)ld8(b), (uint32_t)(ld8(b) >> 32), (uint32_t)ld8(b + 8), (uint32_t)(ld8(b + 8) >> 32)); }
    DW_DEV void st16_both(uint32_t b) const
    {
        const uint64_t lo = ld8(b), hi = ld8(b + 8);
        *reinterpret_cast<uint4 *>(dst + b) = make_uint4((uint32_t)lo, (uint32_t)(lo >> 32), (uint32_t)hi, (uint32_t)(hi >> 32));
        Unal16 v; v.a = lo; v.b = hi; *reinterpret_cast<Unal16 *>(dstb + b) = v;
    }
    DW_DEV void store_range(uint32_t from, uint32_t upto) const { fifo_store_range<BURST>(f, dst, from, upto); }
    DW_DEV void store_range_b(uint32_t from, uint32_t upto) const { fifo_store_range_unaligned<BURST>(f, dstb, from, upto); }
    DW_DEV void drain()
    {
        if (!(probe::off(2))) {
            if (!DUAL) {
                if (skip == 0) { st16(0); st16(16); if (BURST == 64u) { st16(32); st16(48); } }
                else store_range(skip, BURST);
            } else {
                if ((skip | bdone) == 0) { st16_both(0); st16_both(16); if (BURST == 64u) { st16_both(32); st16_both(48); } }
                else {
                    if (skip == 0) { st16(0); st16(16); if (BURST == 64u) { st16(32); st16(48); } } else store_range(skip, BURST);
                    store_range_b(bdone, BURST);
                }
            }
        }
        skip = 0;
        if (DUAL) { bdone = bdone > BURST ? bdone - BURST : 0u; dstb += BURST; }
        *reinterpret_cast<uint64_t *>(f) = ld8(BURST);
        dst += BURST; wp -= BURST;
    }
    DW_DEV void put(uint32_t b) { if (probe::off(1)) return; f[wp] = (uint8_t)b; if (++wp >= BURST) drain(); }
    DW_DEV void putn(uint64_t v, uint32_t cnt)
    {
        if (probe::off(1)) return;
        Unal8 x; x.v = v; *reinterpret_cast<Unal8 *>(f + wp) = x;
        wp += cnt; if (wp >= BURST) drain();
    }
    DW_DEV void poke2(uint32_t off, uint32_t v) { if (probe::off(1)) return; Unal2 x; x.v = (uint16_t)v; *reinterpret_cast<Unal2 *>(f + wp + off) = x; }
    DW_DEV void advance(uint32_t n) { if (probe::off(1)) return; wp += n; if (wp >= BURST) drain(); }
    DW_DEV void put_lead8(uint32_t lead, uint64_t v, uint32_t cnt)
    {
        if (probe::off(1)) return;
        f[wp] = (uint8_t)lead;
        Unal8 x; x.v = v; *reinterpret_cast<Unal8 *>(f + wp + 1) = x;
        wp += cnt + 1; if (wp >= BURST) drain();
    }
    DW_DEV void putn_first_only(uint64_t v, uint32_t cnt, uint32_t only_a)
    {
        if (probe::off(1)) return;
        if (!(probe::off(2))) store_range_b(bdone, wp);
        bdone = wp + only_a; dstb -= only_a;
        putn(v, cnt);
    }
    DW_DEV void put4(uint32_t w) { if (probe::off(1)) return; Unal4 x; x.v = w; *reinterpret_cast<Unal4 *>(f + wp) = x; wp += 4; if (wp >= BURST) drain(); }
    DW_DEV void poke8(uint32_t off, uint64_t v) { if (probe::off(1)) return; Unal8 x; x.v = v; *reinterpret_cast<Unal8 *>(f + wp + off) = x; }
    DW_DEV void poke4(uint32_t off, uint32_t v) { if (probe::off(1)) return; Unal4 x; x.v = v; *reinterpret_cast<Unal4 *>(f + wp + off) = x; }
    DW_DEV void burst32(uint4 lo, uint4 hi)
    {
        static_assert(BURST == 32u && !DUAL, "a unit of two dwordx4 stores, one stream");
        if (probe::off(1)) return;
        if (probe::off(2)) probe::keep(lo.x, lo.y, lo.z, lo.w, hi.x, hi.y, hi.z, hi.w);
        else { *reinterpret_cast<uint4 *>(dst) = lo; *reinterpret_cast<uint4 *>(dst + 16) = hi; }
        dst += 32u;
    }
    DW_DEV void put16(uint32_t a, uint32_t b, uint32_t c, uint32_t d) { putn((uint64_t)a | ((uint64_t)b << 32), 8); putn((uint64_t)c | ((uint64_t)d << 32), 8); }
    DW_DEV void flush()
    {
        if (!(probe::off(2))) { if (wp > skip) store_range(skip, wp); if (DUAL) store_range_b(bdone, wp); }
        dst += wp; if (DUAL) dstb += wp;
        wp = skip = 0; bdone = 0;
    }
};
template <int WR, bool DUAL> struct PrimaryWriter { typedef FifoWriter<32u, DUAL> type; };
template <bool DUAL> struct PrimaryWriter<0, DUAL> { typedef Writer type; };
template <bool DUAL> struct PrimaryWriter<2, DUAL> { typedef FifoWriter<64u, DUAL> type; };
template <int OUT, int WR = 1>
struct Out2 {
    static constexpr bool DUAL = OUT == 3 && WR != 0;
    static constexpr bool TWO = OUT == 3 && WR == 0;
    typename PrimaryWriter<WR, DUAL>::type a; Writer b;
    DW_DEV void init(uint8_t *fifo, uint8_t *bwa, uint8_t *bfast)
    {
        if constexpr (DUAL) a.init(fifo, bwa, bfast);
        else { a.init(fifo, (OUT & 1) ? bwa : bfast); if (TWO) b.init(bfast); }
    }
    DW_DEV void put(uint32_t c) { a.put(c); if (TWO) b.put(c); }
    DW_DEV void put4(uint32_t w) { a.put4(w); if (TWO) b.put4(w); }
    DW_DEV void putn(uint64_t v, uint32_t cnt) { a.putn(v, cnt); if (TWO) b.putn(v, cnt); }
    DW_DEV void put_lead8(uint32_t lead, uint64_t v, uint32_t cnt) { a.put_lead8(lead, v, cnt); if (TWO) b.put_lead8(lead, v, cnt); }
    DW_DEV void put16(uint32_t x, uint32_t y, uint32_t z, uint32_t w) { a.put16(x, y, z, w); if (TWO) b.put16(x, y, z, w); }
    DW_DEV void put_suffix(uint64_t v_bwa, uint32_t n_bwa, uint64_t v_bf, uint32_t n_bf)
    {
        if constexpr (DUAL) a.putn_first_only(v_bwa, n_bwa, n_bwa - n_bf);
        else {
            if (OUT & 1) a.putn(v_bwa, n_bwa); else a.putn(v_bf, n_bf);
            if (TWO) b.putn(v_bf, n_bf);
        }
    }
    DW_DEV void rebase() { if (WR == 0) a.flush(); if (TWO) b.flush(); }
    DW_DEV void flush() { a.flush(); if (TWO) b.flush(); }
};
DW_DEV uint32_t ndigits10(uint32_t v)
{
    return 1u + (v >= 10u) + (v >= 100u) + (v >= 1000u) + (v >= 10000u) + (v >= 100000u) + (v >= 1000000u) + (v >= 10000000u) + (v >= 100000000u) + (v >= 1000000000u);
}
DW_DEV uint32_t ndigits16(uint64_t v) { return v ? (uint32_t)(67 - __clzll((long long)v)) >> 2 : 1u; }
DW_DEV uint32_t dec4(uint32_t x)
{
    const uint32_t a = (x * 5243u) >> 19;
    const uint32_t p = a | ((x - a * 100u) << 16);
    const uint32_t t = ((p * 103u) >> 10) & 0x000F000Fu;
    return (t | ((p - t * 10u) << 8)) + 0x30303030u;
}
DW_DEV uint64_t dec8(uint32_t v)
{
    const uint32_t hi = (uint32_t)(((uint64_t)v * 0xD1B71759ull) >> 45);
    return (uint64_t)dec4(hi) | ((uint64_t)dec4(v - hi * 10000u) << 32);
}
DW_DEV uint64_t dec8_stripped(uint32_t v, uint32_t *nd)
{
    const uint64_t w = dec8(v);
    const uint32_t z = (uint32_t)__builtin_ctzll((w - 0x3030303030303030ull) | (1ull << 56)) >> 3;
    *nd = 8u - z;
    return w >> (8u * z);
}
DW_DEV uint64_t hex8(uint32_t v)
{
    auto four = [](uint32_t n) -> uint32_t {
        uint32_t x = ((n & 0xF000u) >> 12) | ((n & 0x0F00u) << 0) | ((n & 0x00F0u) << 12) | ((n & 0x000Fu) << 24);
        const uint32_t over = ((x + 0x06060606u) >> 4) & 0x01010101u;
        return x + 0x30303030u + over * 39u;
    };
    return (uint64_t)four(v >> 16) | ((uint64_t)four(v & 0xFFFFu) << 32);
}
template <class O>
DW_DEV void put_dec(O &o, uint32_t v, uint32_t lead)
{
    if (v >= 100000000u) {
        const uint32_t hi = v / 100000000u;
        const uint32_t t = (hi * 103u) >> 10;
        o.putn(t ? (uint64_t)lead | ((uint64_t)('0' + t) << 8) | ((uint64_t)('0' + hi - 10u * t) << 16) : (uint64_t)lead | ((uint64_t)('0' + hi) << 8), t ? 3u : 2u);
        o.putn(dec8(v - hi * 100000000u), 8);
        return;
    }
    uint32_t nd; const uint64_t w = dec8_stripped(v, &nd);
    o.put_lead8(lead, w, nd);
}
template <class O>
DW_DEV void put_hex(O &o, uint64_t v, uint32_t lead)
{
    const uint32_t nd = ndigits16(v);
    if (nd > 8) {
        o.put_lead8(lead, hex8((uint32_t)(v >> 32)) >> (8u * (16u - nd)), nd - 8u);
        o.putn(hex8((uint32_t)v), 8);
    } else o.put_lead8(lead, hex8((uint32_t)v) >> (8u * (8u - nd)), nd);
}
template <class O>
DW_DEV void put_counts(O &o, uint32_t e, uint32_t u, uint32_t i)
{
    if (e < 10u && u < 10u && i < 10u)
        o.putn((uint64_t)'_' | ((uint64_t)('0' + e) << 8) | ((uint64_t)':' << 16) | ((uint64_t)('0' + u) << 24) | ((uint64_t)':' << 32) | ((uint64_t)('0' + i) << 40), 6);
    else { put_dec(o, e, '_'); put_dec(o, u, ':'); put_dec(o, i, ':'); }
}
DW_DEV uint32_t counts_len(uint32_t e, uint32_t u, uint32_t i)
{
    return (e < 10u && u < 10u && i < 10u) ? 6u : 3u + ndigits10(e) + ndigits10(u) + ndigits10(i);
}
DW_DEV uint32_t base_chars4(uint32_t nibbles) { return lut8(0x4E4E4E4Eu, 0x54474341u, spread4(nibbles)); }
DW_DEV uint32_t colour_digits4(uint32_t nibbles) { return lut8(0x34343434u, 0x33323130u, spread4(nibbles)); }

}
```

### dwgsim_amd/csrc/dw_simulate.hip

```cpp
#include <algorithm>
#include "dw_read.hpp"
#include "dw_launch.hpp"

#ifndef DW_PART
#define DW_PART -1
#endif
#define DW_HAS(part) (DW_PART == -1 || DW_PART == (part))
#ifndef DW_SIM_WAVES
#define DW_SIM_WAVES 5
#endif
#ifndef DW_SOLID_WAVES
#define DW_SOLID_WAVES 4
#endif
#ifndef DW_SIM_WAVES_BOTH
#define DW_SIM_WAVES_BOTH 4
#endif
#ifndef DW_SIMB_WAVES
#define DW_SIMB_WAVES 6
#endif
#ifndef DW_IONA_WAVES
#define DW_IONA_WAVES 4
#endif
#ifndef DW_IONL_WAVES
#define DW_IONL_WAVES 3
// ... 85 lines not shown
    if (om) {
        const uint32_t li = (blockIdx.x * (PLACE_PAIRS / 64) + (uint32_t)wave) % PLACE_LISTS;
        uint32_t base = 0;
        if (lane == 0) base = atomicAdd(&a.place_list_n[16 * li], (uint32_t)__popcll(om));
        base = (uint32_t)__shfl((int)base, 0);
        const uint32_t at = base + (uint32_t)__popcll(om & ((1ull << lane) - 1ull));
        if (open) {
            if (at < a.place_list_cap) a.place_list[(size_t)li * a.place_list_cap + at] = blockIdx.x * (uint32_t)PLACE_PAIRS + (uint32_t)tid;
            else atomicOr((unsigned long long *)&a.counters[2], 16ull);
        }
    }
    __syncthreads();
    if (tid == 0) { uint32_t t = 0; for (int w = 0; w < PLACE_PAIRS / 64; ++w) t += s_cnt[w]; a.block_rand[blockIdx.x] = t; }
}

__global__ void __launch_bounds__(128) k_place_rest(SimArgs a)
{
    const int lane = (int)(threadIdx.x & 63);
    const uint32_t li = blockIdx.x % PLACE_LISTS, sub = blockIdx.x / PLACE_LISTS, nsub = gridDim.x / PLACE_LISTS;
    uint32_t n = a.place_list_n[16 * li];
    if (n > a.place_list_cap) n = a.place_list_cap;
    for (uint32_t base = sub * 128u; base < n; base += nsub * 128u) {
        const uint32_t q = base + threadIdx.x;
        bool todo = q < n;
        uint32_t e = 0, myseg = 0;
        if (todo) { e = a.place_list[(size_t)li * a.place_list_cap + q]; myseg = seg_of_block(as_constant(a.segs), a.n_seg, e / PLACE_PAIRS); }
        uint32_t retries = 0;
        for (;;) {
            const uint64_t m = __ballot(todo);
            if (!m) break;
            const uint32_t s = uniform_u32((uint32_t)__shfl((int)myseg, __ffsll((unsigned long long)m) - 1));
            if (todo && myseg == s) {
                const SegPtr sg = as_constant(a.segs) + s;
                const SegCtx sc = seg_ctx(a, sg);
                const uint64_t pair = (uint64_t)(e / PLACE_PAIRS - sg->first_block) * PLACE_PAIRS + (uint64_t)(e % PLACE_PAIRS);
                const RngKey key{a.p.seed, uniform_u32(sg->contig_index)};
                bool is_rand, failed; uint32_t att;
                place_pair_exact(a, sc, key, sg->first_ii + pair, is_rand, failed, att);
                if (is_rand) atomicAdd((unsigned long long *)&a.range_rand[s], 1ull);
                if (failed) atomicOr((unsigned long long *)&a.counters[2], 1ull);
                retries = att;
                todo = false;
            }
        }
        const uint32_t rs = wave_sum_u32(retries);
        if (lane == 0 && rs) atomicAdd((unsigned long long *)&a.counters[1], (unsigned long long)rs);
    }
}

__global__ void __launch_bounds__(256) k_range_counts(SimArgs a)
{
    const uint32_t q = blockIdx.x * 256u + threadIdx.x;
    if (q >= (uint32_t)a.n_seg) return;
    const SegPtr sg = as_constant(a.segs);
    const uint64_t lo = a.block_rand[sg[q].first_block], hi = q + 1 < (uint32_t)a.n_seg ? (uint64_t)a.block_rand[sg[q + 1].first_block] : a.counters[3];
    a.range_rand[q] += hi - lo;
    if (q == 0) { uint64_t open = 0; for (int li = 0; li < PLACE_LISTS; ++li) open += a.place_list_n[16 * li]; a.counters[5] = open; }
}
#endif


template <class O>
DW_DEV void put_name_fixed(O &o, const uint32_t *fw, const uint8_t *fx, uint32_t fixed_len)
{
    const uint32_t flen = fixed_len + 1, inl = flen < 128u ? flen : 128u;
    uint32_t q = 0;
    for (; q + 4 <= inl; q += 4) o.put4(fw[q >> 2]);
    if (q < inl) o.putn((uint64_t)fw[q >> 2] & ((1ull << (8 * (inl - q))) - 1), inl - q);
    for (q = inl; q < flen; ++q) o.put(fx[q]);
}
template <class O>
DW_DEV void put_rand_tail(O &o, uint64_t rand_ii)
{
    o.putn(0x305F305F305F305Full, 8);
    o.putn(0x3A305F315F315F00ull >> 8, 7);
    o.putn(0x303A305F303A30ull, 7);
    o.putn(0x303Aull, 2);
    put_hex(o, rand_ii, '_');
}
struct NameCounts { int32_t e0, u0, i0, e1, u1, i1; };
template <class O>
DW_DEV void put_pair_tail(O &o, int32_t x0, int32_t x1, uint32_t strand0, uint32_t strand1, const NameCounts &n, uint64_t ii)
{
    put_dec(o, (uint32_t)(x0 + 1), '_'); put_dec(o, (uint32_t)(x1 + 1), '_');
    o.putn((uint64_t)'_' | ((uint64_t)('0' + strand0) << 8) | ((uint64_t)'_' << 16) | ((uint64_t)('0' + strand1) << 24)
               | ((uint64_t)'_' << 32) | ((uint64_t)'0' << 40) | ((uint64_t)'_' << 48) | ((uint64_t)'0' << 56), 8);
    put_counts(o, (uint32_t)n.e0, (uint32_t)n.u0, (uint32_t)n.i0);
    put_counts(o, (uint32_t)n.e1, (uint32_t)n.u1, (uint32_t)n.i1);
    put_hex(o, ii, '_');
}
DW_DEV uint32_t pair_tail_len(int32_t x0, int32_t x1, const NameCounts &n, uint64_t ii)
{
    return 1 + ndigits10((uint32_t)(x0 + 1)) + 1 + ndigits10((uint32_t)(x1 + 1)) + 8
         + counts_len((uint32_t)n.e0, (uint32_t)n.u0, (uint32_t)n.i0) + counts_len((uint32_t)n.e1, (uint32_t)n.u1, (uint32_t)n.i1) + 1 + ndigits16(ii);
}
DW_DEV void quality_try_exact(uint32_t w, double sigma, bool &ok, int32_t &k0, int32_t &k1)
{
    const double v1 = (double)((int32_t)(w & 0xFFFFu) - 32768) * 0x1p-15, v2 = (double)((int32_t)(w >> 16) - 32768) * 0x1p-15;
    const double rsq = v1 * v1 + v2 * v2;
    ok = !(rsq >= 1.0 || rsq == 0.0);
    if (!ok) return;
    const double fac = sqrt_mid(div_mid(-2.0 * det_log<true>(rsq), rsq));
    k0 = (int32_t)(((v2 * fac) * sigma) + 0.5);
    k1 = (int32_t)(((v1 * fac) * sigma) + 0.5);
}
DW_DEV uint64_t quality_try_exact_called(uint32_t w, double sigma)
{
    bool ok; int32_t k0 = 0, k1 = 0;
    quality_try_exact(w, sigma, ok, k0, k1);
    return (uint64_t)(uint32_t)k0 | ((uint64_t)(uint32_t)k1 << 32);
}
struct QualLazy { float k, eps, lmin; int32_t near1_zero; };
DW_DEV uint32_t quality_try_lazy(uint32_t w, const QualLazy &ql, int32_t &k0, int32_t &k1)
{
    const uint32_t wx = w ^ 0x80008000u;
    const int32_t s1 = (int32_t)(int16_t)(wx & 0xFFFFu), s2 = (int32_t)wx >> 16;
    const uint32_t R = (uint32_t)(s1 * s1) + (uint32_t)(s2 * s2);
    const bool acc = R - 1u < 0x3FFFFFFFu;
    const float Rf = (float)R, rt = Rf * 0x1p-30f;
    const float Lp = -__builtin_amdgcn_logf(rt);
    const float f = __builtin_amdgcn_sqrtf(Lp * __builtin_amdgcn_rcpf(Rf));
    const float y0 = __builtin_fmaf((float)s2 * f, ql.k, 0.5f), y1 = __builtin_fmaf((float)s1 * f, ql.k, 0.5f);
    const float d0 = __builtin_fabsf(y0 - __builtin_rintf(y0)), d1 = __builtin_fabsf(y1 - __builtin_rintf(y1));
    const bool near1 = Lp < ql.lmin;
    const bool sure = near1 ? ql.near1_zero != 0 : (d0 >= ql.eps && d1 >= ql.eps);
    k0 = near1 ? 0 : (int32_t)y0; k1 = near1 ? 0 : (int32_t)y1;
    return (acc ? 1u : 0u) | ((acc && !sure) ? 2u : 0u);
}
DW_DEV uint32_t quality_block(const U4 &b, const QualLazy &ql, double sigma, const uint32_t *qbw, int nq, int pos, uint64_t &blk)
{
    const uint32_t w[4] = {b.x, b.y, b.z, b.w};
    int32_t k[8]; uint32_t acc = 0, need = 0;
#pragma unroll
    for (int t = 0; t < 4; ++t) { const uint32_t r = quality_try_lazy(w[t], ql, k[2 * t], k[2 * t + 1]); acc |= (r & 1u) << t; need |= (r >> 1) << t; }
    if (need) {
#pragma unroll
        for (int t = 0; t < 4; ++t) if ((need >> t) & 1u) { const uint64_t kk = quality_try_exact_called(w[t], sigma); k[2 * t] = (int32_t)(uint32_t)kk; k[2 * t + 1] = (int32_t)(uint32_t)(kk >> 32); }
    }
    const int pc = pos < nq ? pos : nq;
    const uint32_t q0 = qbw[pc >> 2], q1 = qbw[(pc >> 2) + 1], q2 = qbw[(pc >> 2) + 2];
    const uint64_t qb8 = (uint64_t)__builtin_amdgcn_alignbyte(q1, q0, (uint32_t)pc & 3u) | ((uint64_t)__builtin_amdgcn_alignbyte(q2, q1, (uint32_t)pc & 3u) << 32);
    blk = 0; uint32_t nb = 0;
#pragma unroll
    for (int t = 0; t < 4; ++t) {
        const uint32_t qb2 = (uint32_t)(qb8 >> (8 * nb));
        int32_t qa = (int8_t)((int32_t)(int8_t)(qb2 & 0xffu) + k[2 * t]), qc = (int8_t)((int32_t)(int8_t)((qb2 >> 8) & 0xffu) + k[2 * t + 1]);
        qa = qa < 33 ? 33 : qa > 73 ? 73 : qa; qc = qc < 33 ? 33 : qc > 73 ? 73 : qc;
        const bool on = (acc >> t) & 1u;
        blk |= (uint64_t)(on ? ((uint32_t)qa | ((uint32_t)qc << 8)) : 0u) << (8 * nb);
        nb += on ? 2u : 0u;
    }
    return nb;
}
template <class F>
DW_DEV void for_each_quality_block(const SimParams &p, RngKey key, uint32_t dom, uint64_t ii, uint32_t att, const uint32_t *qbw, int nq, int n_chars, bool skip_first, F &&put)
{
    auto deliver = [&](uint64_t blk, uint32_t nb, int pos) {
        if ((int)nb > n_chars - pos) { nb = (uint32_t)(n_chars - pos); blk &= (1ull << (8 * nb)) - 1ull; }
        if (skip_first && pos == 0 && nb) { blk >>= 8; --nb; }
        if (nb) put(blk, nb);
    };
    if (p.fixed_quality >= 0 || !(0 < p.quality_std)) {
        for (int pos = 0; pos < n_chars; pos += 8) {
            uint64_t blk;
            if (p.fixed_quality >= 0) blk = 0x0101010101010101ull * (uint64_t)(uint32_t)p.fixed_quality;
            else {
                const int pc = pos < nq ? pos : nq;
                const uint32_t q0 = qbw[pc >> 2], q1 = qbw[(pc >> 2) + 1], q2 = qbw[(pc >> 2) + 2];
                const uint32_t lo = __builtin_amdgcn_alignbyte(q1, q0, (uint32_t)pc & 3u), hi = __builtin_amdgcn_alignbyte(q2, q1, (uint32_t)pc & 3u);
                blk = 0;
#pragma unroll
                for (int b = 0; b < 8; ++b) { int32_t q = (int8_t)(((b < 4 ? lo : hi) >> (8 * (b & 3))) & 0xffu); q = q < 33 ? 33 : q > 73 ? 73 : q; blk |= (uint64_t)(uint32_t)q << (8 * b); }
            }
            deliver(blk, 8, pos);
        }
        return;
    }
    const QualLazy ql{p.q_k, p.q_eps, p.q_lmin, p.q_near1};
    int pos = 0; uint32_t t = 0;
    while (pos < n_chars) {
        const U4 b = rng_block(key, dom, ii, att, 0, t++);
        uint64_t blk;
        const uint32_t nb = quality_block(b, ql, p.quality_std, qbw, nq, pos, blk);
        deliver(blk, nb, pos);
        pos += (int)nb;
    }
}

DW_DEV uint64_t hex_digits_sum(uint64_t b, uint64_t c)
{
    uint64_t sum = 0;
    for (int d = 1; d <= 16 && c; ++d) {
        const uint64_t hi = d == 16 ? ~0ull : (1ull << (4 * d)) - 1ull;
        if (b > hi) continue;
        const uint64_t n = hi - b + 1ull < c && d < 16 ? hi - b + 1ull : c;
        sum += n * (uint64_t)d; b += n; c -= n;
    }
    return sum;
}
DW_DEV uint32_t scratch_slot_take(uint64_t *ff, uint32_t per_xcd, uint32_t n_blocks)
{
    const uint32_t x = xcc_id();
    const uint64_t q = (uint64_t)atomicAdd((unsigned long long *)&ff[32 * x], 1ull);
    if (q < per_xcd) return x * per_xcd + (uint32_t)q;
    uint64_t *e = ff + 256 + (size_t)x * n_blocks + (size_t)(q - per_xcd);
    uint64_t v;
    do { v = status_load(e); if (v == 0) __builtin_amdgcn_s_sleep(2); } while (v == 0);
    return (uint32_t)(v - 1);
}
DW_DEV void scratch_slot_release(uint64_t *ff, uint32_t n_blocks, uint32_t slot)
{
    const uint32_t x = xcc_id();
    const uint64_t r = (uint64_t)atomicAdd((unsigned long long *)&ff[32 * x + 16], 1ull);
    status_store(ff + 256 + (size_t)x * n_blocks + (size_t)r, (uint64_t)slot + 1ull);
}
constexpr int sim_min_waves(int OUT, int DT, int NTHR, int WR, int SPLIT)
{
    if (DT == 3) return SPLIT == 1 ? DW_IONA_WAVES : SPLIT == 2 ? DW_SIMB_WAVES : DW_IONL_WAVES;
    if (NTHR != SIM_THREADS) return DT == 1 ? DW_SOLID_WAVES : 1;
    if (DT == 2) return DW_ION_WAVES;
    if (DT == 1) return DW_SOLID_WAVES;
    if (SPLIT == 2) return DW_SIMB_WAVES;
    return (OUT != 3 || WR != 0) ? DW_SIM_WAVES : DW_SIM_WAVES_BOTH;
}
template <int LPP, int OUT, int DT, int NTHR, int WR, int SPLIT>
__global__ void __launch_bounds__(NTHR, sim_min_waves(OUT, DT, NTHR, WR, SPLIT)) k_simulate(SimArgs a)
{
    static_assert(SPLIT == 0 || ((DT == 0 || DT == 3) && NTHR == SIM_THREADS), "the two-kernel form exists for the Illumina variants and for Ion Torrent with its buffers in LDS, 256-lane blocks");
    DW_DYN_SHARED(uint32_t, dyn_lds);
    __shared__ uint32_t sm_all[4][16];
    uint32_t (*const sm_bytes)[16] = sm_all, (*const sm_rand)[16] = sm_all + 3, (*const sm_one)[16] = sm_all;
    __shared__ uint32_t s_ticket, s_slot;
    __shared__ uint64_t s_rbase, s_base[3];
    __shared__ uint32_t s_fixed[2][32];
    __shared__ FlowTables s_ft;
    __shared__ uint32_t s_lg[FLOW_LG_ENTRIES];
    constexpr int nthr = NTHR, PPB = NTHR / LPP, nwaves = NTHR / 64;
    constexpr bool ION = DT == 2 || DT == 3;
    constexpr bool GS = DT == 2 || (DT != 3 && NTHR != SIM_THREADS);
    constexpr bool ONE_LB = (DT == 0 || DT == 1) && SPLIT == 0;
    constexpr bool SEQ_LOCKSTEP = DT == 0 && SPLIT == 0 && WR == 1 && NTHR == SIM_THREADS && OUT != 3;
    const int LB_SHIFT = a.lb_shift;
    const int tid = (int)threadIdx.x;
    const int wave = tid >> 6, lane = tid & 63;
    DW_PROBE_INIT();
    if (GS && tid == 0) { s_slot = scratch_slot_take(a.flow_free, (uint32_t)a.flow_slots, a.n_blocks); asm volatile("" ::: "memory"); }
    if (SPLIT == 0 && tid == 0) s_ticket = (uint32_t)atomicAdd((unsigned long long *)&a.counters[0], 1ull);
    if (SPLIT != 1) for (int q = tid; q < 32; q += nthr) s_fixed[1][q] = reinterpret_cast<const uint32_t *>(a.rand_fixed)[q];
    if (ION && tid < 64) s_ft.flow[tid] = a.flow[tid];
    if (!ION && SPLIT != 2) for (int q = tid; q < FLOW_LG_ENTRIES; q += nthr) s_lg[q] = reinterpret_cast<const uint32_t *>(a.flow + 64)[q];
    const size_t stage_words = SPLIT == 2 ? 0 : DT == 3 ? (size_t)(a.lds_words + a.flow_stack_words) : DT == 2 ? (size_t)a.flow_stack_words : GS ? 0 : (size_t)a.lds_words;
    uint32_t *const s_qb = dyn_lds + stage_words * nthr;
    if (SPLIT != 1) for (int q = tid; q < 2 * a.qb_words; q += nthr) s_qb[q] = (q < a.qb_words ? a.qbase[0] : a.qbase[1])[q < a.qb_words ? q : q - a.qb_words];
    uint8_t *const s_fifo = reinterpret_cast<uint8_t *>(dyn_lds + (((stage_words * nthr + 2 * (size_t)a.qb_words) + 3) & ~(size_t)3)) + (size_t)tid * (WR == 2 ? SIM_FIFO_BYTES_WIDE : SIM_FIFO_BYTES);
    if (SPLIT == 0 || (SPLIT == 1 && !ION)) __syncthreads();
    constexpr int H = SPLIT;
    const uint32_t t = SPLIT == 0 ? uniform_u32(s_ticket) : (uint32_t)blockIdx.x;
    const SegPtr sg = as_constant(a.segs) + seg_of_block(as_constant(a.segs), a.n_seg, t);
    const SegCtx sc = seg_ctx(a, sg);
    const uint8_t *name_fixed = a.names + sg->name_off;
    if (H != 1) for (int q = tid; q < 32; q += nthr) s_fixed[0][q] = reinterpret_cast<const uint32_t *>(name_fixed)[q];
    if (ION) { if (SPLIT != 0) __syncthreads(); fill_flow_tables(s_ft, a.flow_len, tid, nthr, a.flow); __syncthreads(); }
    const int j = (LPP == 2) ? (tid & 1) : 0;
    const uint64_t pair_in = (uint64_t)(t - sg->first_block) * PPB + (uint64_t)(tid / LPP);
    const bool valid = pair_in < sg->n_pairs;
    const uint64_t ii = sg->first_ii + pair_in;
    const uint64_t pair = sg->pair_off + pair_in;
    const RngKey key{a.p.seed, uniform_u32(sg->contig_index)};
    const int s = sel_len(a, j);
    uint32_t *lds = GS ? a.flow_scratch + (size_t)uniform_u32(s_slot) * ((size_t)(DT == 2 ? flow_words_per_lane(a.lds_words) : a.lds_words) * nthr) + tid
                  : SPLIT == 2 ? a.split_state + (size_t)t * ((size_t)a.lds_words * nthr) + tid : dyn_lds + tid;
    uint32_t *const flow_stk = dyn_lds + (DT == 3 ? (size_t)a.lds_words * nthr : 0) + tid;
    const int capb = 16 * a.lds_words;

    if (SPLIT == 0) wave_priority(1);
    DW_PROBE_MARK(a, 0);
    PairDraw pd; pd.is_rand = true; pd.pos = pd.d = 0; pd.hap = 0; pd.strand0 = pd.strand1 = 0;
    ReadRes rr{0, 0, 0, 0, 0};
    uint32_t att = 0; bool is_rand = false, done = !valid;
    int32_t n_err = 0;
    int s_out = s;
    bool flow_reversed = false;
    const int nw = (s + 7) >> 3;
    int32_t err_first = 0;
    uint32_t rrank = 0, rtot = 0;
    uint32_t rb[4] = {0, 0, 0, 0};
    if (H != 2) {
    while (__ballot(!done)) {
        bool ok = true;
        if (!done) {
            pd = draw_pair(a, sc, key, ii, att);
            if (pd.is_rand) { is_rand = true; done = true; rr = ReadRes{0, 0, 0, 0, 0}; }
            else if (s > 0) {
                int64_t start; int step;
                read_geom(a, sc, pd, j, &start, &step);
                DW_PROBE_MARK(a, 7);
                if (ION) {
                    const bool rev = (j ? pd.strand1 : pd.strand0) != 0;
                    rr = gen_read(sel_hap(a, sc, pd.hap), sc.l, start, step, s, rev ? 1 : 0, FlowSink{lds, nthr, rev ? (capb >> 3) - 1 : ((capb - s) & ~7) >> 3, rev});
                }
                else if (probe::off(8)) { rr = ReadRes{(int32_t)start, 0, 0, 0, 0}; for (int w = 0; w * 8 < s; ++w) lds[w * nthr] = 0x32103210u; }
                else
                rr = gen_read(sel_hap(a, sc, pd.hap), sc.l, start, step, s, j ? pd.strand1 : pd.strand0, WordSink{lds, nthr});
                ok = rr.ext_coor >= 0 && rr.num_n <= a.p.max_n;
            }
        }
        if (LPP == 2) { const int other = __shfl_xor((int)ok, 1); ok = ok && (other != 0); }
        if (!done) {
            if (ok) done = true;
            else if (++att > (uint32_t)MAX_ATTEMPTS) { atomicOr((unsigned long long *)&a.counters[2], 1ull); done = true; }
        }
    }
    DW_PROBE_MARKF(a, 5);
    if (valid && j == 0) a.meta[pair] = att | (is_rand ? 0x80000000u : 0u) | ((sg->contig_start && pair_in == 0) ? 0x40000000u : 0u);
    { const uint32_t retries = wave_sum_u32((valid && j == 0) ? att : 0u); if (lane == 0 && retries) atomicAdd((unsigned long long *)&a.counters[1], (unsigned long long)retries); }
    if (H == 0 && !ONE_LB) {
    { const uint32_t v[1] = {(is_rand && j == 0) ? 1u : 0u}; uint32_t ex[1], tot[1]; block_excl_scan_n<1>(v, sm_rand, ex, tot); rrank = ex[0]; rtot = tot[0]; }
    DW_PROBE_MARKF(a, 6);
    if (wave == 0) {
        const uint64_t g = probe::off(128) ? (uint64_t)t * 6 : lookback_excl(a.status[2], t, rtot, 0);
        if (lane == 0) { s_rbase = g; if (t + 1 == a.n_blocks) a.counters[3] = g + rtot; }
    }
    }
    DW_PROBE_MARK(a, 1);
    if (ION) {
        const bool flows = valid && !is_rand && s > 0;
        FlowRng rg; rg.seed = key.seed; rg.contig = key.contig; rg.dom = D_FLOW0 + (uint32_t)j; rg.att = att; rg.evt = 0; rg.s = 0; rg.ii = ii; rg.w0 = rg.w1 = rg.w2 = rg.w3 = 0;
        const int so = flow_errors(flows, rg, s_ft, a.flow_len, (j ? a.e_thr[1] : a.e_thr[0])[0], j ? a.flow_gap_r[1] : a.flow_gap_r[0], j ? a.flow_gap_s[1] : a.flow_gap_s[0], lds, flow_stk, nthr, 2 * a.flow_stack_words, s, j ? pd.strand1 : pd.strand0, capb, &n_err);
        if (flows) {
            s_out = so;
            if (s_out < 0) { atomicOr((unsigned long long *)&a.counters[2], 2ull); s_out = 0; }
            flow_reversed = (j ? pd.strand1 : pd.strand0) != 0;
        }
    }
    if (ION) {
        if (valid && is_rand) for (int w = 0; w * 16 < s; ++w) {
            if ((w & 3) == 0) { const U4 q0 = rng_block(key, D_BASE0 + (uint32_t)j, ii, att, 0, (uint32_t)(w >> 2)); rb[0] = q0.x; rb[1] = q0.y; rb[2] = q0.z; rb[3] = q0.w; }
            uint32_t pairs = (w & 2) ? ((w & 1) ? rb[3] : rb[2]) : ((w & 1) ? rb[1] : rb[0]);
            const int rem = s - 16 * w;
            if (rem < 16) pairs &= (1u << (2 * rem)) - 1u;
            lds[w * nthr] = pairs;
        }
    } else
    if (valid && !(probe::off(4))) {
        if (is_rand) {
            uint32_t prev_base = 0;
            for (int w = 0; w < nw; ++w) {
                if ((w & 7) == 0) { const U4 q0 = rng_block(key, D_BASE0 + (uint32_t)j, ii, att, 0, (uint32_t)(w >> 3)); rb[0] = q0.x; rb[1] = q0.y; rb[2] = q0.z; rb[3] = q0.w; }
                const uint32_t wd = ((w >> 1) & 2) ? (((w >> 1) & 1) ? rb[3] : rb[2]) : (((w >> 1) & 1) ? rb[1] : rb[0]);
                uint32_t word = pairs_to_nibbles((wd >> (16 * (w & 1))) & 0xFFFFu);
                const int rem = s - 8 * w;
                const uint32_t live = rem >= 8 ? 0xFFFFFFFFu : ((1u << (4 * rem)) - 1u);
                if (DT == 1) {
                    const uint32_t prevw = (word << 4) | prev_base;
                    prev_base = word >> 28;
                    word = (word ^ prevw) & 0x33333333u;
                }
                lds[w * nthr] = word & live;
            }
        } else {
            if (DT == 1) {
                uint32_t prev_base = 0;
                for (int w = 0; w < nw; ++w) {
                    uint32_t word = lds[w * nthr];
                    const uint32_t prevw = (word << 4) | prev_base;
                    prev_base = word >> 28;
                    const uint32_t n = (word | prevw) & 0x44444444u;
                    word = ((word ^ prevw) & 0x33333333u & ~((n >> 1) | (n >> 2))) | n;
                    const int rem = s - 8 * w;
                    lds[w * nthr] = rem >= 8 ? word : word & ((1u << (4 * rem)) - 1u);
                }
            }
            const uint64_t tmax = j ? a.err_thr_max[1] : a.err_thr_max[0], gR = j ? a.err_gap_r[1] : a.err_gap_r[0];
            const int gS = j ? a.err_gap_s[1] : a.err_gap_s[0]; const bool ramp = (j ? a.err_ramp[1] : a.err_ramp[0]) != 0;
            const uint64_t *thr64 = j ? a.e_thr[1] : a.e_thr[0];
            if (tmax) {
                uint32_t m = 0, S = 0, tw[4] = {0, 0, 0, 0}, sw[4] = {0, 0, 0, 0};
                for (;;) {
                    if ((m & 3u) == 0u) {
                        const U4 q0 = rng_block(key, D_BASE0 + (uint32_t)j, ii, att, 0, m >> 2); rb[0] = q0.x; rb[1] = q0.y; rb[2] = q0.z; rb[3] = q0.w;
                        if (ramp) { const U4 q1 = rng_block(key, D_BASE_REF0 + (uint32_t)j, ii, att, 0, m >> 2); tw[0] = q1.x; tw[1] = q1.y; tw[2] = q1.z; tw[3] = q1.w; }
                    }
                    const uint32_t k4 = m & 3u;
                    const uint32_t gw = (k4 & 2u) ? ((k4 & 1u) ? rb[3] : rb[2]) : ((k4 & 1u) ? rb[1] : rb[0]);
                    const uint32_t G = tmax >= 0x100000000ull ? 0u : geom_gap(gw, s_lg, gR, gS);
                    S = m ? S + 1u + G : G;
                    if (S >= (uint32_t)s) break;
                    if (k4 == 0u) { const U4 q2 = rng_block(key, D_SUB0 + (uint32_t)j, ii, att, 0, m >> 2); sw[0] = q2.x; sw[1] = q2.y; sw[2] = q2.z; sw[3] = q2.w; }
                    const int w = (int)(S >> 3), sh = 4 * (int)(S & 7u);
                    const uint32_t word = lds[w * nthr];
                    bool hit = ((word >> sh) & 4u) == 0u;
                    if (ramp && hit) {
                        const uint64_t ti = thr64[S];
                        const uint32_t w2 = (k4 & 2u) ? ((k4 & 1u) ? tw[3] : tw[2]) : ((k4 & 1u) ? tw[1] : tw[0]);
                        hit = ti >= tmax || (uint64_t)w2 * tmax < (ti << 32);
                    }
                    if (hit) {
                        const uint32_t rwd = (k4 & 2u) ? ((k4 & 1u) ? sw[3] : sw[2]) : ((k4 & 1u) ? sw[1] : sw[0]);
                        const uint32_t add = 1u + (uint32_t)(((uint64_t)rwd * 3u) >> 32);
                        const uint32_t c = (((word >> sh) & 3u) + add) & 3u;
                        lds[w * nthr] = (word & ~(0xFu << sh)) | (c << sh);
                        ++n_err; if (DT == 1 && S == 0u) err_first = 1;
                    }
                    ++m;
                }
            }
        }
    }
    }
    uint64_t pre_rand = 0, pre_b1 = 0, pre_b2 = 0;
    if (SPLIT == 2) {
        const uint64_t *pi = a.split_pre + 4 * (size_t)t, *pc = a.split_chunk + 4 * (size_t)(t >> 10);
        pre_rand = pi[0] + pc[0];
        const uint64_t hexb = hex_digits_sum(a.chain[0], pre_rand);
        pre_b1 = pi[1] + pc[1] + hexb; pre_b2 = pi[2] + pc[2] + (LPP == 2 ? hexb : 0ull);
    }
    if (ION && H == 2 && (a.counters[2] & 2ull)) return;
    if (H == 2) {
        const uint4 hm = reinterpret_cast<const uint4 *>(a.split_hand)[(size_t)t * nthr + tid];
        rr.ext_coor = (int32_t)hm.x; n_err = (int32_t)(hm.y & 0xffffu); rr.n_sub = (int32_t)(hm.y >> 16); rr.n_indel = (int32_t)(hm.z & 0xffffu); rr.n_ins = (int32_t)(hm.z >> 16);
        att = hm.w & 0x3fffu; is_rand = (hm.w >> 14) & 1u; pd.strand0 = (int)((hm.w >> 15) & 1u); pd.strand1 = (int)((hm.w >> 16) & 1u);
        if (ION) { s_out = (int)(hm.w >> 17); flow_reversed = !is_rand && (j ? pd.strand1 : pd.strand0) != 0; }
        __syncthreads();
        { const uint32_t v[1] = {(is_rand && j == 0) ? 1u : 0u}; uint32_t ex[1], tot[1]; block_excl_scan_n<1>(v, sm_rand, ex, tot); rrank = ex[0]; rtot = tot[0]; }
    }
    DW_PROBE_MARKF(a, 2);
    if (H == 0 && !ONE_LB) __syncthreads();
    uint64_t rand_ii = (H == 1 || ONE_LB) ? 0 : a.chain[0] + (SPLIT == 2 ? pre_rand : s_rbase) + rrank - ((LPP == 2 && j == 1 && is_rand) ? 1u : 0u);
    DW_PROBE_MARK(a, 2);
    int32_t e0 = n_err, u0 = rr.n_sub, i0 = rr.n_indel, x0 = rr.ext_coor;
    int32_t e1c = 0, u1 = 0, i1 = 0, x1 = 0;
    if (LPP == 2) {
        const int32_t o0 = __shfl_xor(n_err, 1), o1 = __shfl_xor(rr.n_sub, 1), o2 = __shfl_xor(rr.n_indel, 1), o3 = __shfl_xor(rr.ext_coor, 1);
        if (j == 0) { e1c = o0; u1 = o1; i1 = o2; x1 = o3; }
        else { e1c = n_err; u1 = rr.n_sub; i1 = rr.n_indel; x1 = rr.ext_coor; e0 = o0; u0 = o1; i0 = o2; x0 = o3; }
    }
    int32_t e0w = e0, i0w = i0, e1w = e1c, i1w = i1;
    if (DT == 1) {
        int32_t f0 = err_first, g0 = rr.n_ins, f1 = 0, g1 = 0;
        if (LPP == 2) {
            const int32_t of = __shfl_xor(err_first, 1), og = __shfl_xor(rr.n_ins, 1);
            if (j == 0) { f1 = of; g1 = og; } else { f1 = err_first; g1 = rr.n_ins; f0 = of; g0 = og; }
        }
        e0w = e0 - f0; i0w = i0 - g0; e1w = e1c - f1; i1w = i1 - g1;
    }
    const NameCounts nc{e0, u0, i0, e1c, u1, i1}, ncw{e0w, u0, i0w, e1w, u1, i1w};
    uint32_t tail_len, tail_len_w, fixed_len;
    if (is_rand) { fixed_len = (uint32_t)a.rand_fixed_len; tail_len = tail_len_w = 25u + ((H == 1 || ONE_LB) ? 0u : ndigits16(rand_ii)); }
    else {
        fixed_len = (uint32_t)sg->name_fixed_len;
        tail_len = pair_tail_len(x0, x1, nc, ii);
        tail_len_w = (DT == 1) ? pair_tail_len(x0, x1, ncw, ii) : tail_len;
    }
    const bool emits = valid && s_out > 0;
    const uint32_t Lbwa = !emits ? 0u : (DT == 1) ? (1u + fixed_len + tail_len_w + 2u + 1u + 2u * (uint32_t)(s_out - 1) + 3u + 1u)
                                                  : (1u + fixed_len + tail_len + 2u + 1u + (uint32_t)s_out + 3u + (uint32_t)s_out + 1u);

    constexpr bool BF_SCAN = DT != 0 && SPLIT == 0;
    uint32_t e1, e2, eb = 0, T1, T2, Tb = 0;
    uint64_t G1_one = 0, G2_one = 0, Gb_one = 0;
    if (ONE_LB) {
        constexpr bool BF_ONE = DT == 1;
        constexpr int NS = BF_ONE ? 4 : 3;
        const uint32_t Lbf1 = (BF_ONE && emits) ? (1u + fixed_len + tail_len + 1u + 1u + 2u * (uint32_t)s_out + 3u + 1u) : 0u;
        uint32_t v[NS], ex[NS], tot[NS];
        v[0] = (is_rand && j == 0) ? 1u : 0u; v[1] = j == 0 ? Lbwa : 0u; v[2] = j == 1 ? Lbwa : 0u; if (BF_ONE) v[NS - 1] = Lbf1;
        block_excl_scan_n<NS>(v, sm_one, ex, tot);
        rrank = ex[0]; e1 = ex[1]; e2 = ex[2]; rtot = tot[0]; if (BF_ONE) eb = ex[NS - 1];
        DW_PROBE_MARKF(a, 6);
        if (wave == 0) {
            const uint64_t g = lookback_excl(a.status[0], t, ((uint64_t)tot[0] << LB_SHIFT) | (uint64_t)tot[1], 0);
            if (lane == 0) s_base[0] = g;
        }
        if (BF_ONE && wave == (nwaves > 1 ? 1 : 0)) { const uint64_t gb = lookback_excl(a.status[3], t, (uint64_t)tot[NS - 1], 0); if (lane == 0) s_base[2] = gb; }
        __syncthreads();
        const uint64_t pk = s_base[0];
        const uint64_t base_r = pk >> LB_SHIFT, pre1 = pk & ((1ull << LB_SHIFT) - 1ull);
        const uint64_t rb0 = a.chain[0] + base_r;
        const uint64_t hex_before = hex_digits_sum(a.chain[0], base_r);
        const uint64_t pairs_before = sg->pair_off + (uint64_t)(t - sg->first_block) * PPB;
        G1_one = pre1 + hex_before;
        G2_one = LPP == 2 ? pre1 + (uint64_t)((int64_t)2 * (a.p.len[1] - a.p.len[0]) * (int64_t)pairs_before) + hex_before : 0ull;
        const uint32_t cnt2 = rrank - ((LPP == 2 && j == 1 && is_rand) ? 1u : 0u);
        rand_ii = rb0 + cnt2;
        if (is_rand) tail_len = tail_len_w = 25u + ndigits16(rand_ii);
        const uint32_t dlo = ndigits16(rb0);
        const bool one_width = dlo == ndigits16(rb0 + rtot);
        const uint32_t h1 = one_width ? dlo * rrank : (uint32_t)hex_digits_sum(rb0, rrank), h2 = one_width ? dlo * cnt2 : (uint32_t)hex_digits_sum(rb0, cnt2);
        const uint32_t htot = one_width ? dlo * rtot : (uint32_t)hex_digits_sum(rb0, rtot);
        e1 += h1; if (LPP == 2) e2 += h2;
        T1 = tot[1] + htot; T2 = tot[2] + (LPP == 2 ? htot : 0u);
        if (BF_ONE) {
            eb += LPP == 2 ? h1 + h2 : h1; Tb = tot[NS - 1] + (LPP == 2 ? 2u : 1u) * htot;
            Gb_one = s_base[2] + (LPP == 2 ? 2ull : 1ull) * hex_before;
        }
        if (tid == nthr - 1 && t + 1 == a.n_blocks) a.counters[3] = base_r + rtot;
    } else
    if (BF_SCAN) {
        const uint32_t Lbf = !emits ? 0u : DT == 1 ? (1u + fixed_len + tail_len + 1u + 1u + 2u * (uint32_t)s_out + 3u + 1u) : Lbwa - 2u;
        const uint32_t v[3] = {j == 0 ? Lbwa : 0u, j == 1 ? Lbwa : 0u, Lbf};
        uint32_t ex[3], tot[3]; block_excl_scan_n<3>(v, sm_bytes, ex, tot);
        e1 = ex[0]; e2 = ex[1]; eb = ex[2]; T1 = tot[0]; T2 = tot[1]; Tb = tot[2];
    } else if (H != 1) {
        const uint32_t v[2] = {j == 0 ? Lbwa : 0u, j == 1 ? Lbwa : 0u};
        uint32_t ex[2], tot[2]; block_excl_scan_n<2>(v, sm_bytes, ex, tot);
        e1 = ex[0]; e2 = ex[1]; T1 = tot[0]; T2 = tot[1];
    } else { e1 = e2 = T1 = T2 = 0; }
    if (H == 1) {
        const uint32_t rsum = wave_sum_u32((is_rand && j == 0) ? 1u : 0u), b1 = wave_sum_u32(j == 0 ? Lbwa : 0u), b2 = wave_sum_u32(j == 1 ? Lbwa : 0u);
        if (lane == 0) { sm_rand[0][wave] = rsum; sm_bytes[0][wave] = b1; sm_bytes[1][wave] = b2; }
        const uint4 hm = make_uint4((uint32_t)rr.ext_coor, (uint32_t)n_err | ((uint32_t)rr.n_sub << 16), (uint32_t)rr.n_indel | ((uint32_t)rr.n_ins << 16),
                                    att | (is_rand ? 1u << 14 : 0u) | ((uint32_t)pd.strand0 << 15) | ((uint32_t)pd.strand1 << 16) | (ION ? (uint32_t)s_out << 17 : 0u));
        reinterpret_cast<uint4 *>(a.split_hand)[(size_t)t * nthr + tid] = hm;
        uint32_t *gs = a.split_state + (size_t)t * ((size_t)a.lds_words * nthr) + tid;
        if (valid) for (int w = 0, n_w = ION ? (s_out + 15) >> 4 : nw; w < n_w; ++w) gs[(size_t)w * nthr] = lds[w * nthr];
        __syncthreads();
        if (tid == 0) { uint32_t r = 0, t1 = 0, t2 = 0; for (int w = 0; w < nwaves; ++w) { r += sm_rand[0][w]; t1 += sm_bytes[0][w]; t2 += sm_bytes[1][w]; } reinterpret_cast<uint4 *>(a.split_agg)[t] = make_uint4(r, t1, t2, 0u); }
        return;
    }
    if (H == 0 && !ONE_LB) {
    if (wave == 0) {
        const uint64_t g = probe::off(128) ? (uint64_t)t * PPB * (uint64_t)(60 + 2 * s + a.rand_fixed_len + sg->name_fixed_len) : lookback_excl(a.status[0], t, T1, 0); if (lane == 0) s_base[0] = g;
        if (BF_SCAN) { const uint64_t gb = lookback_excl(a.status[3], t, Tb, 0); if (lane == 0) s_base[2] = gb; }
    }
    if (wave == (nwaves > 1 ? 1 : 0)) { const uint64_t g = probe::off(128) ? (uint64_t)t * PPB * (uint64_t)(60 + 2 * s + a.rand_fixed_len + sg->name_fixed_len) : lookback_excl(a.status[1], t, T2, 0); if (lane == 0) s_base[1] = g; }
    __syncthreads();
    }
    const uint64_t G1 = ONE_LB ? G1_one : SPLIT == 2 ? pre_b1 : s_base[0], G2 = ONE_LB ? G2_one : SPLIT == 2 ? pre_b2 : s_base[1];
    const uint64_t reads_before_block = (sg->pair_off + (uint64_t)(t - sg->first_block) * PPB) * (uint64_t)LPP;
    const uint64_t nvalid_before = (uint64_t)tid;
    const uint64_t off_bwa = (j == 0) ? G1 + e1 : G2 + e2;
    const uint64_t off_bf = BF_SCAN ? (ONE_LB ? Gb_one : s_base[2]) + eb : G1 + G2 - 2 * reads_before_block + e1 + e2 - 2 * nvalid_before;
    if (H == 0 && tid == nthr - 1) {
        if (t + 1 == a.n_blocks) {
            const uint64_t nreads = a.n_pairs * (uint64_t)((a.p.len[1] > 0) ? 2 : 1);
            a.counters[4] = a.p.has_bwa ? G1 + T1 : 0;
            a.counters[5] = a.p.has_bwa ? G2 + T2 : 0;
            a.counters[6] = !a.p.has_bfast ? 0 : BF_SCAN ? (ONE_LB ? Gb_one : s_base[2]) + Tb : G1 + T1 + G2 + T2 - 2 * nreads;
        }
    }

    if (SPLIT == 0 && DT == 1) wave_priority(0);
    DW_PROBE_MARK(a, 3);
    if (DT == 1) {
        if (emits) {
            for (int which = 0; which < 2; ++which) {
                if (!(OUT & (1 << which))) continue;
                Out2<1, WR> o;
                o.init(s_fifo, which ? a.out[2] + off_bf : (j ? a.out[1] : a.out[0]) + off_bwa, nullptr);
                put_name_fixed(o, is_rand ? s_fixed[1] : s_fixed[0], is_rand ? a.rand_fixed : name_fixed, fixed_len);
                if (is_rand) put_rand_tail(o, rand_ii);
                else put_pair_tail(o, x0, x1, pd.strand0, pd.strand1,
                                   NameCounts{which ? e0 : e0w, u0, which ? i0 : i0w, which ? e1c : e1w, u1, which ? i1 : i1w}, ii);
                if (which == 0) o.putn((uint64_t)'/' | ((uint64_t)('2' - j) << 8) | ((uint64_t)'\n' << 16), 3);
                else { o.put('\n'); o.put('A'); }
                const int first = which ? 0 : 1;
                for (int w = 0; w * 8 < s_out; ++w) {
                    const uint32_t word = lds[w * nthr];
                    const uint32_t c0 = which ? colour_digits4(word) : base_chars4(word), c1 = which ? colour_digits4(word >> 16) : base_chars4(word >> 16);
                    const int lo = w == 0 ? first : 0, hi = s_out - w * 8 < 8 ? s_out - w * 8 : 8;
                    if (lo == 0 && hi == 8) { o.put4(c0); o.put4(c1); }
                    else for (int b = lo; b < hi; ++b) o.put(((b < 4 ? c0 : c1) >> (8 * (b & 3))) & 0xff);
                }
                o.put('\n'); o.put('+'); o.put('\n');
                for_each_quality_block(a.p, key, D_QUAL0 + (uint32_t)j, ii, att, s_qb + (j ? a.qb_words : 0), s, s_out, first != 0,
                                       [&](uint64_t blk, uint32_t nb) { o.putn(blk, nb); });
                o.put('\n');
                o.flush();
            }
        }
    } else
    {
        const bool rec = valid && s_out > 0;
        Out2<OUT, WR> o;
        if (rec) {
        o.init(s_fifo, (OUT & 1) ? (j ? a.out[1] : a.out[0]) + off_bwa : nullptr, (OUT & 2) ? a.out[2] + off_bf : nullptr);
        if (!(probe::off(16))) {
        put_name_fixed(o, is_rand ? s_fixed[1] : s_fixed[0], is_rand ? a.rand_fixed : name_fixed, fixed_len);
        if (is_rand) put_rand_tail(o, rand_ii);
        else put_pair_tail(o, x0, x1, pd.strand0, pd.strand1, nc, ii);
        }
        o.put_suffix((uint64_t)'/' | ((uint64_t)('1' + j) << 8) | ((uint64_t)'\n' << 16), 3, (uint64_t)'\n', 1);
        if (SPLIT == 0) wave_priority(0);
        DW_PROBE_MARK(a, 4);
        o.rebase();
        auto rec_word = [&](int w) -> uint32_t {
            if (!ION) return lds[w * nthr];
            const Buf2 B{lds, nthr, a.lds_words};
            if (!flow_reversed) return pairs_to_nibbles(B.get8(8 * w));
            const int lo = s_out - 8 - 8 * w;
            return pairs_to_nibbles(lo < 0 ? reverse_pairs16(B.get8(0)) >> (2 * (-lo)) : reverse_pairs16(B.get8(lo)));
        };
        auto put_last_word = [&](uint32_t word, int rem) __attribute__((always_inline)) {
            if (rem >= 8) { o.put4(base_chars4(word)); o.put4(base_chars4(word >> 16)); }
            else { const uint32_t c0 = base_chars4(word), c1 = base_chars4(word >> 16); for (int b = 0; b < rem; ++b) o.put(((b < 4 ? c0 : c1) >> (8 * (b & 3))) & 0xff); }
        };
        if (SPLIT == 2 && !ION) {
            const int full16 = s_out >> 4;
            for (int g0 = 0; g0 < full16; g0 += 4) {
                uint32_t r[8];
#pragma unroll
                for (int k = 0; k < 8; ++k) r[k] = (g0 + (k >> 1) < full16) ? lds[(size_t)(2 * g0 + k) * nthr] : 0u;
#pragma unroll
                for (int q = 0; q < 4; ++q) if (g0 + q < full16) o.put16(base_chars4(r[2 * q]), base_chars4(r[2 * q] >> 16), base_chars4(r[2 * q + 1]), base_chars4(r[2 * q + 1] >> 16));
            }
            if (s_out & 15) {
                const int w = 2 * full16, rem = s_out - 8 * w;
                const uint32_t wa = lds[(size_t)w * nthr], wb = rem > 8 ? lds[(size_t)(w + 1) * nthr] : 0u;
                put_last_word(wa, rem);
                if (rem > 8) put_last_word(wb, rem - 8);
            }
        } else if (ION) {
            const Buf2 B{lds, nthr, a.lds_words};
            const int full16 = s_out >> 4;
            const uint32_t sh2 = ((uint32_t)s_out & 15u) * 2u;
            for (int g0 = 0; g0 < full16; g0 += 4) {
                uint32_t r[5];
                const int base = flow_reversed ? ((s_out - 16 * g0) >> 4) - 4 : g0;
#pragma unroll
                for (int q = 0; q < 5; ++q) r[q] = (base + q >= 0 && (flow_reversed || q < 4)) ? B.word(base + q) : 0u;
#pragma unroll
                for (int k = 0; k < 4; ++k) if (g0 + k < full16) {
                    uint32_t v;
                    if (!flow_reversed) v = r[k];
                    else {
                        v = sh2 ? __builtin_amdgcn_alignbit(r[4 - k], r[3 - k], sh2) : r[3 - k];
                        v = __builtin_bitreverse32(v); v = ((v & 0x55555555u) << 1) | ((v >> 1) & 0x55555555u);
                    }
                    const uint32_t n0 = pairs_to_nibbles(v & 0xFFFFu), n1 = pairs_to_nibbles(v >> 16);
                    o.put16(base_chars4(n0), base_chars4(n0 >> 16), base_chars4(n1), base_chars4(n1 >> 16));
                }
            }
            for (int w = 2 * full16; w * 8 < s_out; ++w) put_last_word(rec_word(w), s_out - w * 8);
        } else if constexpr (SEQ_LOCKSTEP) {
            auto &fw = o.a;
            auto staged = [&](int w) -> uint32_t { return w < nw ? lds[w * nthr] : 0u; };
            auto chars8 = [&](uint32_t nib) -> uint64_t { return (uint64_t)base_chars4(nib) | ((uint64_t)base_chars4(nib >> 16) << 32); };
            const int na = s_out < 32 - (int)fw.wp ? s_out : 32 - (int)fw.wp;
#pragma unroll
            for (int k = 0; k < 4; ++k) if (8 * k < na) fw.poke8(8u * (uint32_t)k, chars8(lds[k * nthr]));
            fw.advance((uint32_t)na);
            const uint32_t sh = 4u * ((uint32_t)na & 7u);
            const int left = s_out - na, rem = left & 31;
            int wi = na >> 3;
            uint32_t r0 = left > 0 ? staged(wi) : 0u;
            for (int c = left >> 5; c > 0; --c, wi += 4) {
                const uint32_t r1 = lds[(wi + 1) * nthr], r2 = lds[(wi + 2) * nthr], r3 = lds[(wi + 3) * nthr], r4 = staged(wi + 4);
                const uint32_t n0 = __builtin_amdgcn_alignbit(r1, r0, sh), n1 = __builtin_amdgcn_alignbit(r2, r1, sh);
                const uint32_t n2 = __builtin_amdgcn_alignbit(r3, r2, sh), n3 = __builtin_amdgcn_alignbit(r4, r3, sh);
                fw.burst32(make_uint4(base_chars4(n0), base_chars4(n0 >> 16), base_chars4(n1), base_chars4(n1 >> 16)),
                           make_uint4(base_chars4(n2), base_chars4(n2 >> 16), base_chars4(n3), base_chars4(n3 >> 16)));
                r0 = r4;
            }
#pragma unroll
            for (int k = 0; k < 4; ++k) if (8 * k < rem) {
                const uint32_t r1 = staged(wi + k + 1);
                fw.poke8(8u * (uint32_t)k, chars8(__builtin_amdgcn_alignbit(r1, r0, sh)));
                r0 = r1;
            }
            fw.poke4((uint32_t)rem, (uint32_t)'\n' | ((uint32_t)'+' << 8) | ((uint32_t)'\n' << 16));
            fw.advance((uint32_t)rem + 3u);
        } else {
        int w = 0;
        for (; (w + 2) * 8 <= s_out; w += 2) {
            const uint32_t w0 = rec_word(w), w1 = rec_word(w + 1);
            o.put16(base_chars4(w0), base_chars4(w0 >> 16), base_chars4(w1), base_chars4(w1 >> 16));
        }
        for (; w * 8 < s_out; ++w) put_last_word(rec_word(w), s_out - w * 8);
        }
        if constexpr (!SEQ_LOCKSTEP) { o.put('\n'); o.put('+'); o.put('\n'); }
        o.rebase();
        }
        if (SPLIT == 0) wave_priority(0);
        DW_PROBE_MARK(a, 5);
        if (rec) {
            for_each_quality_block(a.p, key, D_QUAL0 + (uint32_t)j, ii, att, s_qb + (j ? a.qb_words : 0), s, s_out, false, [&](uint64_t blk, uint32_t nb) { o.putn(blk, nb); });
        }
        if (rec) { o.put('\n'); o.flush(); }
    }
    DW_PROBE_MARK(a, 6);
    if (GS) {
        wait_stores();
        __syncthreads();
        if (tid == 0) scratch_slot_release(a.flow_free, a.n_blocks, s_slot);
    }
}

#if DW_HAS(0)
__global__ void __launch_bounds__(256) k_selftest_fp64(uint32_t seed, uint64_t n, uint64_t *mism)
{
    const uint64_t i = (uint64_t)blockIdx.x * 256 + threadIdx.x;
    uint32_t bad_div = 0, bad_sqrt = 0, bad_log = 0, done = 0;
    if (i < n) {
        const RngKey key{seed, 0u};
        const U4 b = rng_block(key, 31, i, 0, 0, 0), c = rng_block(key, 31, i, 0, 0, 1);
        const double a1 = (double)b.x * 0x1p-31 - 1.0, a2 = (double)b.y * 0x1p-31 - 1.0, r = a1 * a1 + a2 * a2;
        if (r < 1.0 && r != 0.0) {
            const double l1 = det_log(r), l2 = det_log<true>(r);
            bad_log += dbl_bits(l1) != dbl_bits(l2);
            const double x = -2.0 * l1, q1 = x / r, q2 = div_mid(x, r);
            bad_div += dbl_bits(q1) != dbl_bits(q2);
            bad_sqrt += dbl_bits(sqrt(q1)) != dbl_bits(sqrt_mid(q1));
            const double f = bits_dbl((dbl_bits(r) & 0x000FFFFFFFFFFFFFull) | 0x3FF0000000000000ull) - 1.0;
            bad_div += dbl_bits(f / (2.0 + f)) != dbl_bits(div_mid(f, 2.0 + f));
            done += 4;
        }
        {
            const double p1 = 2.0 * u53(c.x, c.y) - 1.0, p2 = 2.0 * u53(c.z, c.w) - 1.0, pr = p1 * p1 + p2 * p2;
            if (pr < 1.0 && pr >= 0x1p-60) {
                const double l1 = det_log(pr), l2 = det_log<true>(pr);
                bad_log += dbl_bits(l1) != dbl_bits(l2);
                const double q1 = (-2.0 * l1) / pr;
                bad_div += dbl_bits(q1) != dbl_bits(div_mid(-2.0 * l1, pr));
                bad_sqrt += dbl_bits(sqrt(q1)) != dbl_bits(sqrt_mid(q1));
                done += 3;
            }
        }
        const double x = ldexp(1.0 + u53(c.x, c.y), (int)(b.z % 141u) - 70), y = ldexp(1.0 + u53(c.z, c.w), (int)(b.w % 141u) - 70);
        bad_div += dbl_bits(x / y) != dbl_bits(div_mid(x, y));
        bad_sqrt += dbl_bits(sqrt(x)) != dbl_bits(sqrt_mid(x));
        done += 2;
    }
    const uint32_t s0 = wave_sum_u32(bad_div), s1 = wave_sum_u32(bad_sqrt), s2 = wave_sum_u32(bad_log), s3 = wave_sum_u32(done);
    if ((threadIdx.x & 63) == 0) {
        if (s0) atomicAdd((unsigned long long *)&mism[0], (unsigned long long)s0);
        if (s1) atomicAdd((unsigned long long *)&mism[1], (unsigned long long)s1);
        if (s2) atomicAdd((unsigned long long *)&mism[2], (unsigned long long)s2);
        atomicAdd((unsigned long long *)&mism[3], (unsigned long long)s3);
    }
}
DW_DEV void atomic_max_pos_double(uint64_t *p, double v) { atomicMax((unsigned long long *)p, (unsigned long long)dbl_bits(v)); }
__global__ void __launch_bounds__(256) k_selftest_lazy(int mode, uint32_t first, uint64_t n, double sigma, float qk, float qeps, float qlmin, int qnear1, uint64_t *out)
{
    uint32_t bad_k = 0, bad_acc = 0, n_fast = 0, n_slow = 0, n_all = 0; double worst = 0.0;
    for (uint64_t i = (uint64_t)blockIdx.x * 256 + threadIdx.x; i < n; i += (uint64_t)gridDim.x * 256) {
        if (mode == 0) {
            const uint32_t w = first + (uint32_t)i;
            const QualLazy ql{qk, qeps, qlmin, qnear1};
            int32_t k0 = 0, k1 = 0, e0 = 0, e1 = 0; bool eok = false;
            const uint32_t r = quality_try_lazy(w, ql, k0, k1);
            quality_try_exact(w, sigma, eok, e0, e1);
            ++n_all;
            if ((r & 1u) != (eok ? 1u : 0u)) ++bad_acc;
            else if (eok) {
                if (r & 2u) ++n_slow;
                else {
                    ++n_fast;
                    bad_k += (k0 != e0) + (k1 != e1);
                    const int32_t s1 = (int32_t)(w & 0xFFFFu) - 32768, s2 = (int32_t)(w >> 16) - 32768;
                    const double v1 = (double)s1 * 0x1p-15, v2 = (double)s2 * 0x1p-15, rsq = v1 * v1 + v2 * v2;
                    const double fac = sqrt(-2.0 * det_log(rsq) / rsq);
                    const float Rf = (float)((uint32_t)(s1 * s1) + (uint32_t)(s2 * s2)), Lp = -__builtin_amdgcn_logf(Rf * 0x1p-30f);
                    if (!(Lp < ql.lmin)) {
                        const float f = __builtin_amdgcn_sqrtf(Lp * __builtin_amdgcn_rcpf(Rf));
                        const double y0 = (double)__builtin_fmaf((float)s2 * f, ql.k, 0.5f), y1 = (double)__builtin_fmaf((float)s1 * f, ql.k, 0.5f);
                        const double d0 = fabs(y0 - ((v2 * fac) * sigma + 0.5)), d1 = fabs(y1 - ((v1 * fac) * sigma + 0.5));
                        const double wv = (d0 > d1 ? d0 : d1) / (double)ql.eps;
                        worst = wv > worst ? wv : worst;
                    }
                }
            }
        } else {
            const uint32_t base = mode == 1 ? 0x30800000u : mode == 2 ? 0x3F800000u : 0x2B000000u;
            union { uint32_t u; float f; } c; c.u = base + (uint32_t)i;
            const double x = (double)c.f;
            double e;
            if (mode == 1) { const double t = det_log(x) * 1.44269504088896340736; e = fabs((double)__builtin_amdgcn_logf(c.f) - t) / (0x1p-23 * (1.0 + fabs(t))); }
            else if (mode == 2) { const double t = 1.0 / x; e = fabs((double)__builtin_amdgcn_rcpf(c.f) - t) / t / 0x1p-23; }
            else { const double t = sqrt(x); e = fabs((double)__builtin_amdgcn_sqrtf(c.f) - t) / t / 0x1p-23; }
            worst = e > worst ? e : worst;
        }
    }
    const uint32_t s0 = wave_sum_u32(bad_k), s1 = wave_sum_u32(bad_acc), s2 = wave_sum_u32(n_fast), s3 = wave_sum_u32(n_slow), s4 = wave_sum_u32(n_all);
    if ((threadIdx.x & 63) == 0) {
        if (s0) atomicAdd((unsigned long long *)&out[0], (unsigned long long)s0);
        if (s1) atomicAdd((unsigned long long *)&out[1], (unsigned long long)s1);
        atomicAdd((unsigned long long *)&out[2], (unsigned long long)s2);
        atomicAdd((unsigned long long *)&out[3], (unsigned long long)s3);
        atomicAdd((unsigned long long *)&out[4], (unsigned long long)s4);
    }
    if (worst > 0.0) atomic_max_pos_double(&out[mode == 0 ? 5 : 5 + mode], worst);
}
void launch_selftest_lazy(hipStream_t st, int mode, uint32_t first, uint64_t n, double sigma, float qk, float qeps, float qlmin, int qnear1, uint64_t *out)
{
    const uint64_t nb = (n + 255) / 256;
    hipLaunchKernelGGL(k_selftest_lazy, dim3((uint32_t)(nb < (1u << 20) ? (nb ? nb : 1) : (1u << 20))), dim3(256), 0, st, mode, first, n, sigma, qk, qeps, qlmin, qnear1, out);
}
struct TextCollect {
    uint8_t b[24]; uint32_t n;
    DW_DEV void putn(uint64_t v, uint32_t cnt) { for (uint32_t k = 0; k < cnt; ++k) b[n++] = (uint8_t)(v >> (8 * k)); }
    DW_DEV void put_lead8(uint32_t lead, uint64_t v, uint32_t cnt) { b[n++] = (uint8_t)lead; putn(v, cnt); }
};
__global__ void __launch_bounds__(256) k_selftest_text(uint64_t first, uint64_t n, uint64_t stride, uint64_t *out)
{
    uint32_t bad_dec = 0, bad_hex = 0, done = 0;
    for (uint64_t i = (uint64_t)blockIdx.x * 256 + threadIdx.x; i < n; i += (uint64_t)gridDim.x * 256) {
        const uint64_t v = first + i * stride;
        uint8_t want[24]; uint32_t wn;
        { uint8_t d[10]; uint32_t nd = 0, t = (uint32_t)v; do { d[nd++] = (uint8_t)('0' + t % 10u); t /= 10u; } while (t); wn = 0; want[wn++] = '_'; while (nd) want[wn++] = d[--nd]; }
        TextCollect c; c.n = 0;
        put_dec(c, (uint32_t)v, '_');
        bool same = c.n == wn && wn == 1u + ndigits10((uint32_t)v);
        for (uint32_t k = 0; k < wn && same; ++k) same = c.b[k] == want[k];
        bad_dec += same ? 0u : 1u;
        { uint8_t d[16]; uint32_t nd = 0; uint64_t t = v; do { const uint32_t h = (uint32_t)(t & 15u); d[nd++] = (uint8_t)(h < 10 ? '0' + h : 'a' + (h - 10)); t >>= 4; } while (t); wn = 0; want[wn++] = ':'; while (nd) want[wn++] = d[--nd]; }
        c.n = 0;
        put_hex(c, v, ':');
        same = c.n == wn && wn == 1u + ndigits16(v);
        for (uint32_t k = 0; k < wn && same; ++k) same = c.b[k] == want[k];
        bad_hex += same ? 0u : 1u;
        ++done;
    }
    if (bad_dec) atomicAdd((unsigned long long *)&out[0], (unsigned long long)bad_dec);
    if (bad_hex) atomicAdd((unsigned long long *)&out[1], (unsigned long long)bad_hex);
    atomicAdd((unsigned long long *)&out[2], (unsigned long long)done);
}
void launch_selftest_text(hipStream_t st, uint64_t first, uint64_t n, uint64_t stride, uint64_t *out)
{
    const uint64_t nb = cdiv(n, 256);
    hipLaunchKernelGGL(k_selftest_text, dim3((uint32_t)(nb < (1u << 16) ? (nb ? nb : 1) : (1u << 16))), dim3(256), 0, st, first, n, stride, out);
}
constexpr uint32_t GAP_RUN = 256;
__global__ void __launch_bounds__(256) k_selftest_gap(const uint32_t *lg, uint64_t R, int sR, uint32_t first, uint64_t n, uint32_t g_lo, uint32_t g_cnt, uint32_t *chg, uint64_t *out)
{
    __shared__ uint32_t s_lg[FLOW_LG_ENTRIES];
    for (int q = threadIdx.x; q < FLOW_LG_ENTRIES; q += 256) s_lg[q] = lg[q];
    __syncthreads();
    uint32_t up = 0, clip = 0, done = 0;
    const uint64_t g_end = (uint64_t)g_lo + g_cnt;
    for (uint64_t r = (uint64_t)blockIdx.x * 256 + threadIdx.x; r * GAP_RUN < n; r += (uint64_t)gridDim.x * 256) {
        const uint64_t i0 = r * GAP_RUN, i1 = i0 + GAP_RUN < n ? i0 + GAP_RUN : n;
// ... 327 lines not shown
```

Before: 1463.

## Stream quality lines through per-lane LDS rows with wave-uniform 32-byte units

Changes the lockstep sequence staging layout from block-strided to wave-local strided, so each lane's staged words sit inside a per-wave region. After the sequence is written, that region is reused as a contiguous per-lane row buffer for the quality line. Quality blocks are appended unaligned and drained as aligned 32-byte dwordx4 units at regular trip counts, instead of going through the generic FIFO putn/flush path. The diff also fixes the byte offset of a final partial sink put. It adds an extra ballot and carries the risk of LDS aliasing between the staged sequence and the quality rows.

New measurement: 1523, median of 6. 1.04x the previous value.

```diff
diff --git a/dwgsim_amd/csrc/dw_host.cpp b/dwgsim_amd/csrc/dw_host.cpp
--- a/dwgsim_amd/csrc/dw_host.cpp
+++ b/dwgsim_amd/csrc/dw_host.cpp
@@ -151,7 +151,7 @@
     int flow_cap_mult = 1;
     int ion_lds = -1;
     int n_cu = 0; int flow_slots = 0;
-    int64_t walk_cap = -1; bool phases = false; int writer = -1, force_threads = 0; int64_t place_cap = -1; uint64_t place_open = 0; double walk_us = 0, count_us = 0; int split = -1;
+    int64_t walk_cap = -1; bool phases = false; int writer = -1, force_threads = 0; int64_t place_cap = -1; uint64_t place_open = 0; double walk_us = 0, count_us = 0; int split = -1, qrows = 1;
     int64_t sim_form = 0;
     int64_t walk_form = 0;
     hipEvent_t ev_cnt0 = nullptr, ev_cnt1 = nullptr;
@@ -1613,6 +1613,7 @@
     a.rand_fixed = c->d_rand_fixed.get(); a.rand_fixed_len = c->rand_fixed_len;
     a.sim_threads = f.nthr; a.fifo = f.wr != 0; a.split = f.split; a.ion_lds = f.dt == 3;
     a.cap = f.cap; a.lds_words = f.lds_words; a.flow_stack_words = f.stack_words;
+    a.qrows = (c->qrows != 0 && f.dt == 0 && f.split == 0 && f.wr == 1 && f.nthr == SIM_THREADS && f.out != 3 && f.lds_words >= 18) ? 1 : 0;
     a.flow = c->d_flow.get(); a.flow_len = (int32_t)c->flow.size();
     for (int j = 0; j < 2; ++j) {
         const int n = c->prm.length[j];
@@ -2075,6 +2076,7 @@
     else if (!strcmp(key, "walk_seg_min")) walk_debug_seg_min((uint32_t)value);
     else if (!strcmp(key, "place_cap")) c->place_cap = value;
     else if (!strcmp(key, "split")) c->split = (int)value;
+    else if (!strcmp(key, "qrows")) c->qrows = (int)value;
     else if (!strcmp(key, "flow_slots")) c->flow_slots = (int)value;
     else if (!strcmp(key, "ion_lds")) c->ion_lds = (int)value;
     else if (!strcmp(key, "flow_cap")) c->flow_cap_forced = (int)value;
diff --git a/dwgsim_amd/csrc/dw_kernels.hpp b/dwgsim_amd/csrc/dw_kernels.hpp
--- a/dwgsim_amd/csrc/dw_kernels.hpp
+++ b/dwgsim_amd/csrc/dw_kernels.hpp
@@ -191,6 +191,7 @@
     const uint8_t *flow;
     uint64_t flow_gap_r[2]; int32_t flow_gap_s[2];
     uint64_t err_thr_max[2], err_gap_r[2]; int32_t err_gap_s[2], err_ramp[2];
+    int32_t qrows;
 };
 
 }
diff --git a/dwgsim_amd/csrc/dw_read.hpp b/dwgsim_amd/csrc/dw_read.hpp
--- a/dwgsim_amd/csrc/dw_read.hpp
+++ b/dwgsim_amd/csrc/dw_read.hpp
@@ -140,7 +140,7 @@
         if (k < 0) break;
     }
     if (k != s) { r.ext_coor = -10; return r; }
-    if (na) sink.put(k >> 3, accw, na);
+    if (na) sink.put((k - na) >> 3, accw, na);
     return r;
 }
 
@@ -622,10 +622,12 @@
         lo = hi = 0; n = 0;
     }
 };
-template <uint32_t BURST>
+struct Al8 { uint64_t v; };
+struct __attribute__((packed, aligned(4))) Al4x8 { uint64_t v; };
+template <uint32_t BURST, class L8 = Al8>
 DW_DEV void fifo_store_range(const uint8_t *f, uint8_t *dst, uint32_t from, uint32_t upto)
 {
-    auto ld8 = [&](uint32_t b) { return *reinterpret_cast<const uint64_t *>(f + b); };
+    auto ld8 = [&](uint32_t b) { return reinterpret_cast<const L8 *>(f + b)->v; };
     auto st16 = [&](uint32_t b) { *reinterpret_cast<uint4 *>(dst + b) = make_uint4((uint32_t)ld8(b), (uint32_t)(ld8(b) >> 32), (uint32_t)ld8(b + 8), (uint32_t)(ld8(b + 8) >> 32)); };
     uint32_t b = from;
     if ((b & 1u) && b + 1 <= upto) { dst[b] = f[b]; b += 1; }
@@ -724,6 +726,35 @@
         dst += 32u;
     }
     DW_DEV void put16(uint32_t a, uint32_t b, uint32_t c, uint32_t d) { putn((uint64_t)a | ((uint64_t)b << 32), 8); putn((uint64_t)c | ((uint64_t)d << 32), 8); }
+    DW_DEV void rows_take(uint8_t *row)
+    {
+        static_assert(BURST == 32u && !DUAL, "a unit of two dwordx4 stores, one stream");
+        if (!(probe::off(1))) {
+#pragma unroll
+            for (uint32_t b = 0; b < 32u; b += 8u) { Al4x8 x; x.v = ld8(b); *reinterpret_cast<Al4x8 *>(row + b) = x; }
+        }
+        f = row; skip = 0;
+    }
+    DW_DEV void rows_append(uint64_t v, uint32_t cnt) { if (probe::off(1)) return; Unal8 x; x.v = v; *reinterpret_cast<Unal8 *>(f + wp) = x; wp += cnt; }
+    DW_DEV void rows_unit()
+    {
+        auto ld = [&](uint32_t b) { return reinterpret_cast<const Al4x8 *>(f + b)->v; };
+        if (!(probe::off(2))) {
+            const uint64_t a = ld(0), b = ld(8), c = ld(16), d = ld(24);
+            *reinterpret_cast<uint4 *>(dst) = make_uint4((uint32_t)a, (uint32_t)(a >> 32), (uint32_t)b, (uint32_t)(b >> 32));
+            *reinterpret_cast<uint4 *>(dst + 16) = make_uint4((uint32_t)c, (uint32_t)(c >> 32), (uint32_t)d, (uint32_t)(d >> 32));
+        }
+        const uint64_t t0 = ld(32), t1 = ld(40), t2 = ld(48), t3 = ld(56);
+        Al4x8 x;
+        x.v = t0; *reinterpret_cast<Al4x8 *>(f) = x; x.v = t1; *reinterpret_cast<Al4x8 *>(f + 8) = x;
+        x.v = t2; *reinterpret_cast<Al4x8 *>(f + 16) = x; x.v = t3; *reinterpret_cast<Al4x8 *>(f + 24) = x;
+        dst += 32u; wp -= 32u;
+    }
+    DW_DEV void rows_flush()
+    {
+        if (!(probe::off(2))) { if (wp) fifo_store_range<BURST, Al4x8>(f, dst, 0u, wp); }
+        dst += wp; wp = skip = 0;
+    }
     DW_DEV void flush()
     {
         if (!(probe::off(2))) { if (wp > skip) store_range(skip, wp); if (DUAL) store_range_b(bdone, wp); }
diff --git a/dwgsim_amd/csrc/dw_simulate.hip b/dwgsim_amd/csrc/dw_simulate.hip
--- a/dwgsim_amd/csrc/dw_simulate.hip
+++ b/dwgsim_amd/csrc/dw_simulate.hip
@@ -261,8 +261,8 @@
     }
     return nb;
 }
-template <class F>
-DW_DEV void for_each_quality_block(const SimParams &p, RngKey key, uint32_t dom, uint64_t ii, uint32_t att, const uint32_t *qbw, int nq, int n_chars, bool skip_first, F &&put)
+template <class F, class T>
+DW_DEV void for_each_quality_block(const SimParams &p, RngKey key, uint32_t dom, uint64_t ii, uint32_t att, const uint32_t *qbw, int nq, int n_chars, bool skip_first, F &&put, T &&trip)
 {
     auto deliver = [&](uint64_t blk, uint32_t nb, int pos) {
         if ((int)nb > n_chars - pos) { nb = (uint32_t)(n_chars - pos); blk &= (1ull << (8 * nb)) - 1ull; }
@@ -282,6 +282,7 @@
                 for (int b = 0; b < 8; ++b) { int32_t q = (int8_t)(((b < 4 ? lo : hi) >> (8 * (b & 3))) & 0xffu); q = q < 33 ? 33 : q > 73 ? 73 : q; blk |= (uint64_t)(uint32_t)q << (8 * b); }
             }
             deliver(blk, 8, pos);
+            trip((uint32_t)(pos >> 3) + 1u);
         }
         return;
     }
@@ -293,7 +294,13 @@
         const uint32_t nb = quality_block(b, ql, p.quality_std, qbw, nq, pos, blk);
         deliver(blk, nb, pos);
         pos += (int)nb;
-    }
+        trip(t);
+    }
+}
+template <class F>
+DW_DEV void for_each_quality_block(const SimParams &p, RngKey key, uint32_t dom, uint64_t ii, uint32_t att, const uint32_t *qbw, int nq, int n_chars, bool skip_first, F &&put)
+{
+    for_each_quality_block(p, key, dom, ii, att, qbw, nq, n_chars, skip_first, put, [](uint32_t) {});
 }
 
 DW_DEV uint64_t hex_digits_sum(uint64_t b, uint64_t c)
@@ -349,6 +356,7 @@
     constexpr bool GS = DT == 2 || (DT != 3 && NTHR != SIM_THREADS);
     constexpr bool ONE_LB = (DT == 0 || DT == 1) && SPLIT == 0;
     constexpr bool SEQ_LOCKSTEP = DT == 0 && SPLIT == 0 && WR == 1 && NTHR == SIM_THREADS && OUT != 3;
+    constexpr int LSTR = SEQ_LOCKSTEP ? 64 : NTHR;
     const int LB_SHIFT = a.lb_shift;
     const int tid = (int)threadIdx.x;
     const int wave = tid >> 6, lane = tid & 63;
@@ -361,7 +369,7 @@
     const size_t stage_words = SPLIT == 2 ? 0 : DT == 3 ? (size_t)(a.lds_words + a.flow_stack_words) : DT == 2 ? (size_t)a.flow_stack_words : GS ? 0 : (size_t)a.lds_words;
     uint32_t *const s_qb = dyn_lds + stage_words * nthr;
     if (SPLIT != 1) for (int q = tid; q < 2 * a.qb_words; q += nthr) s_qb[q] = (q < a.qb_words ? a.qbase[0] : a.qbase[1])[q < a.qb_words ? q : q - a.qb_words];
-    uint8_t *const s_fifo = reinterpret_cast<uint8_t *>(dyn_lds + (((stage_words * nthr + 2 * (size_t)a.qb_words) + 3) & ~(size_t)3)) + (size_t)tid * (WR == 2 ? SIM_FIFO_BYTES_WIDE : SIM_FIFO_BYTES);
+    auto lane_fifo = [&]() { return reinterpret_cast<uint8_t *>(dyn_lds + (((stage_words * nthr + 2 * (size_t)a.qb_words) + 3) & ~(size_t)3)) + (size_t)tid * (WR == 2 ? SIM_FIFO_BYTES_WIDE : SIM_FIFO_BYTES); };
     if (SPLIT == 0 || (SPLIT == 1 && !ION)) __syncthreads();
     constexpr int H = SPLIT;
     const uint32_t t = SPLIT == 0 ? uniform_u32(s_ticket) : (uint32_t)blockIdx.x;
@@ -378,7 +386,7 @@
     const RngKey key{a.p.seed, uniform_u32(sg->contig_index)};
     const int s = sel_len(a, j);
     uint32_t *lds = GS ? a.flow_scratch + (size_t)uniform_u32(s_slot) * ((size_t)(DT == 2 ? flow_words_per_lane(a.lds_words) : a.lds_words) * nthr) + tid
-                  : SPLIT == 2 ? a.split_state + (size_t)t * ((size_t)a.lds_words * nthr) + tid : dyn_lds + tid;
+                  : SPLIT == 2 ? a.split_state + (size_t)t * ((size_t)a.lds_words * nthr) + tid : SEQ_LOCKSTEP ? dyn_lds + wave * (a.lds_words * 64) + lane : dyn_lds + tid;
     uint32_t *const flow_stk = dyn_lds + (DT == 3 ? (size_t)a.lds_words * nthr : 0) + tid;
     const int capb = 16 * a.lds_words;
 
@@ -408,9 +416,9 @@
                     const bool rev = (j ? pd.strand1 : pd.strand0) != 0;
                     rr = gen_read(sel_hap(a, sc, pd.hap), sc.l, start, step, s, rev ? 1 : 0, FlowSink{lds, nthr, rev ? (capb >> 3) - 1 : ((capb - s) & ~7) >> 3, rev});
                 }
-                else if (probe::off(8)) { rr = ReadRes{(int32_t)start, 0, 0, 0, 0}; for (int w = 0; w * 8 < s; ++w) lds[w * nthr] = 0x32103210u; }
+                else if (probe::off(8)) { rr = ReadRes{(int32_t)start, 0, 0, 0, 0}; for (int w = 0; w * 8 < s; ++w) lds[w * LSTR] = 0x32103210u; }
                 else
-                rr = gen_read(sel_hap(a, sc, pd.hap), sc.l, start, step, s, j ? pd.strand1 : pd.strand0, WordSink{lds, nthr});
+                rr = gen_read(sel_hap(a, sc, pd.hap), sc.l, start, step, s, j ? pd.strand1 : pd.strand0, WordSink{lds, LSTR});
                 ok = rr.ext_coor >= 0 && rr.num_n <= a.p.max_n;
             }
         }
@@ -448,7 +456,7 @@
             uint32_t pairs = (w & 2) ? ((w & 1) ? rb[3] : rb[2]) : ((w & 1) ? rb[1] : rb[0]);
             const int rem = s - 16 * w;
             if (rem < 16) pairs &= (1u << (2 * rem)) - 1u;
-            lds[w * nthr] = pairs;
+            lds[w * LSTR] = pairs;
         }
     } else
     if (valid && !(probe::off(4))) {
@@ -465,19 +473,19 @@
                     prev_base = word >> 28;
                     word = (word ^ prevw) & 0x33333333u;
                 }
-                lds[w * nthr] = word & live;
+                lds[w * LSTR] = word & live;
             }
         } else {
             if (DT == 1) {
                 uint32_t prev_base = 0;
                 for (int w = 0; w < nw; ++w) {
-                    uint32_t word = lds[w * nthr];
+                    uint32_t word = lds[w * LSTR];
                     const uint32_t prevw = (word << 4) | prev_base;
                     prev_base = word >> 28;
                     const uint32_t n = (word | prevw) & 0x44444444u;
                     word = ((word ^ prevw) & 0x33333333u & ~((n >> 1) | (n >> 2))) | n;
                     const int rem = s - 8 * w;
-                    lds[w * nthr] = rem >= 8 ? word : word & ((1u << (4 * rem)) - 1u);
+                    lds[w * LSTR] = rem >= 8 ? word : word & ((1u << (4 * rem)) - 1u);
                 }
             }
             const uint64_t tmax = j ? a.err_thr_max[1] : a.err_thr_max[0], gR = j ? a.err_gap_r[1] : a.err_gap_r[0];
@@ -497,7 +505,7 @@
                     if (S >= (uint32_t)s) break;
                     if (k4 == 0u) { const U4 q2 = rng_block(key, D_SUB0 + (uint32_t)j, ii, att, 0, m >> 2); sw[0] = q2.x; sw[1] = q2.y; sw[2] = q2.z; sw[3] = q2.w; }
                     const int w = (int)(S >> 3), sh = 4 * (int)(S & 7u);
-                    const uint32_t word = lds[w * nthr];
+                    const uint32_t word = lds[w * LSTR];
                     bool hit = ((word >> sh) & 4u) == 0u;
                     if (ramp && hit) {
                         const uint64_t ti = thr64[S];
@@ -508,7 +516,7 @@
                         const uint32_t rwd = (k4 & 2u) ? ((k4 & 1u) ? sw[3] : sw[2]) : ((k4 & 1u) ? sw[1] : sw[0]);
                         const uint32_t add = 1u + (uint32_t)(((uint64_t)rwd * 3u) >> 32);
                         const uint32_t c = (((word >> sh) & 3u) + add) & 3u;
-                        lds[w * nthr] = (word & ~(0xFu << sh)) | (c << sh);
+                        lds[w * LSTR] = (word & ~(0xFu << sh)) | (c << sh);
                         ++n_err; if (DT == 1 && S == 0u) err_first = 1;
                     }
                     ++m;
@@ -622,7 +630,7 @@
                                     att | (is_rand ? 1u << 14 : 0u) | ((uint32_t)pd.strand0 << 15) | ((uint32_t)pd.strand1 << 16) | (ION ? (uint32_t)s_out << 17 : 0u));
         reinterpret_cast<uint4 *>(a.split_hand)[(size_t)t * nthr + tid] = hm;
         uint32_t *gs = a.split_state + (size_t)t * ((size_t)a.lds_words * nthr) + tid;
-        if (valid) for (int w = 0, n_w = ION ? (s_out + 15) >> 4 : nw; w < n_w; ++w) gs[(size_t)w * nthr] = lds[w * nthr];
+        if (valid) for (int w = 0, n_w = ION ? (s_out + 15) >> 4 : nw; w < n_w; ++w) gs[(size_t)w * nthr] = lds[w * LSTR];
         __syncthreads();
         if (tid == 0) { uint32_t r = 0, t1 = 0, t2 = 0; for (int w = 0; w < nwaves; ++w) { r += sm_rand[0][w]; t1 += sm_bytes[0][w]; t2 += sm_bytes[1][w]; } reinterpret_cast<uint4 *>(a.split_agg)[t] = make_uint4(r, t1, t2, 0u); }
         return;
@@ -656,7 +664,7 @@
             for (int which = 0; which < 2; ++which) {
                 if (!(OUT & (1 << which))) continue;
                 Out2<1, WR> o;
-                o.init(s_fifo, which ? a.out[2] + off_bf : (j ? a.out[1] : a.out[0]) + off_bwa, nullptr);
+                o.init(lane_fifo(), which ? a.out[2] + off_bf : (j ? a.out[1] : a.out[0]) + off_bwa, nullptr);
                 put_name_fixed(o, is_rand ? s_fixed[1] : s_fixed[0], is_rand ? a.rand_fixed : name_fixed, fixed_len);
                 if (is_rand) put_rand_tail(o, rand_ii);
                 else put_pair_tail(o, x0, x1, pd.strand0, pd.strand1,
@@ -665,7 +673,7 @@
                 else { o.put('\n'); o.put('A'); }
                 const int first = which ? 0 : 1;
                 for (int w = 0; w * 8 < s_out; ++w) {
-                    const uint32_t word = lds[w * nthr];
+                    const uint32_t word = lds[w * LSTR];
                     const uint32_t c0 = which ? colour_digits4(word) : base_chars4(word), c1 = which ? colour_digits4(word >> 16) : base_chars4(word >> 16);
                     const int lo = w == 0 ? first : 0, hi = s_out - w * 8 < 8 ? s_out - w * 8 : 8;
                     if (lo == 0 && hi == 8) { o.put4(c0); o.put4(c1); }
@@ -683,7 +691,7 @@
         const bool rec = valid && s_out > 0;
         Out2<OUT, WR> o;
         if (rec) {
-        o.init(s_fifo, (OUT & 1) ? (j ? a.out[1] : a.out[0]) + off_bwa : nullptr, (OUT & 2) ? a.out[2] + off_bf : nullptr);
+        o.init(lane_fifo(), (OUT & 1) ? (j ? a.out[1] : a.out[0]) + off_bwa : nullptr, (OUT & 2) ? a.out[2] + off_bf : nullptr);
         if (!(probe::off(16))) {
         put_name_fixed(o, is_rand ? s_fixed[1] : s_fixed[0], is_rand ? a.rand_fixed : name_fixed, fixed_len);
         if (is_rand) put_rand_tail(o, rand_ii);
@@ -694,7 +702,7 @@
         DW_PROBE_MARK(a, 4);
         o.rebase();
         auto rec_word = [&](int w) -> uint32_t {
-            if (!ION) return lds[w * nthr];
+            if (!ION) return lds[w * LSTR];
             const Buf2 B{lds, nthr, a.lds_words};
             if (!flow_reversed) return pairs_to_nibbles(B.get8(8 * w));
             const int lo = s_out - 8 - 8 * w;
@@ -709,13 +717,13 @@
             for (int g0 = 0; g0 < full16; g0 += 4) {
                 uint32_t r[8];
 #pragma unroll
-                for (int k = 0; k < 8; ++k) r[k] = (g0 + (k >> 1) < full16) ? lds[(size_t)(2 * g0 + k) * nthr] : 0u;
+                for (int k = 0; k < 8; ++k) r[k] = (g0 + (k >> 1) < full16) ? lds[(size_t)(2 * g0 + k) * LSTR] : 0u;
 #pragma unroll
                 for (int q = 0; q < 4; ++q) if (g0 + q < full16) o.put16(base_chars4(r[2 * q]), base_chars4(r[2 * q] >> 16), base_chars4(r[2 * q + 1]), base_chars4(r[2 * q + 1] >> 16));
             }
             if (s_out & 15) {
                 const int w = 2 * full16, rem = s_out - 8 * w;
-                const uint32_t wa = lds[(size_t)w * nthr], wb = rem > 8 ? lds[(size_t)(w + 1) * nthr] : 0u;
+                const uint32_t wa = lds[(size_t)w * LSTR], wb = rem > 8 ? lds[(size_t)(w + 1) * LSTR] : 0u;
                 put_last_word(wa, rem);
                 if (rem > 8) put_last_word(wb, rem - 8);
             }
@@ -743,18 +751,18 @@
             for (int w = 2 * full16; w * 8 < s_out; ++w) put_last_word(rec_word(w), s_out - w * 8);
         } else if constexpr (SEQ_LOCKSTEP) {
             auto &fw = o.a;
-            auto staged = [&](int w) -> uint32_t { return w < nw ? lds[w * nthr] : 0u; };
+            auto staged = [&](int w) -> uint32_t { return w < nw ? lds[w * LSTR] : 0u; };
             auto chars8 = [&](uint32_t nib) -> uint64_t { return (uint64_t)base_chars4(nib) | ((uint64_t)base_chars4(nib >> 16) << 32); };
             const int na = s_out < 32 - (int)fw.wp ? s_out : 32 - (int)fw.wp;
 #pragma unroll
-            for (int k = 0; k < 4; ++k) if (8 * k < na) fw.poke8(8u * (uint32_t)k, chars8(lds[k * nthr]));
+            for (int k = 0; k < 4; ++k) if (8 * k < na) fw.poke8(8u * (uint32_t)k, chars8(lds[k * LSTR]));
             fw.advance((uint32_t)na);
             const uint32_t sh = 4u * ((uint32_t)na & 7u);
             const int left = s_out - na, rem = left & 31;
             int wi = na >> 3;
             uint32_t r0 = left > 0 ? staged(wi) : 0u;
             for (int c = left >> 5; c > 0; --c, wi += 4) {
-                const uint32_t r1 = lds[(wi + 1) * nthr], r2 = lds[(wi + 2) * nthr], r3 = lds[(wi + 3) * nthr], r4 = staged(wi + 4);
+                const uint32_t r1 = lds[(wi + 1) * LSTR], r2 = lds[(wi + 2) * LSTR], r3 = lds[(wi + 3) * LSTR], r4 = staged(wi + 4);
                 const uint32_t n0 = __builtin_amdgcn_alignbit(r1, r0, sh), n1 = __builtin_amdgcn_alignbit(r2, r1, sh);
                 const uint32_t n2 = __builtin_amdgcn_alignbit(r3, r2, sh), n3 = __builtin_amdgcn_alignbit(r4, r3, sh);
                 fw.burst32(make_uint4(base_chars4(n0), base_chars4(n0 >> 16), base_chars4(n1), base_chars4(n1 >> 16)),
@@ -782,10 +790,32 @@
         }
         if (SPLIT == 0) wave_priority(0);
         DW_PROBE_MARK(a, 5);
+        bool rows = false;
+        if constexpr (SEQ_LOCKSTEP) {
+            if (a.qrows) {
+                asm volatile("" ::: "memory");
+                rows = __ballot(rec && o.a.skip != 0u) == 0;
+                asm volatile("" ::: "memory");
+            }
+        }
+        if (SEQ_LOCKSTEP && rows) {
+            if constexpr (SEQ_LOCKSTEP) if (rec) {
+                auto &fw = o.a;
+                const uint32_t at = (uint32_t)(lds - dyn_lds);
+                fw.rows_take(reinterpret_cast<uint8_t *>(dyn_lds + (at & ~63u)) + (at & 63u) * (4u * (uint32_t)a.lds_words));
+                for_each_quality_block(a.p, key, D_QUAL0 + (uint32_t)j, ii, att, s_qb + (j ? a.qb_words : 0), s, s_out, false,
+                                       [&](uint64_t blk, uint32_t nb) { fw.rows_append(blk, nb); },
+                                       [&](uint32_t trips) { if ((trips & 3u) == 0u) { if (fw.wp >= 32u) fw.rows_unit(); } });
+                fw.rows_append((uint64_t)'\n', 1);
+                if (fw.wp >= 32u) fw.rows_unit();
+                fw.rows_flush();
+            }
+        } else {
         if (rec) {
             for_each_quality_block(a.p, key, D_QUAL0 + (uint32_t)j, ii, att, s_qb + (j ? a.qb_words : 0), s, s_out, false, [&](uint64_t blk, uint32_t nb) { o.putn(blk, nb); });
         }
         if (rec) { o.put('\n'); o.flush(); }
+        }
     }
     DW_PROBE_MARK(a, 6);
     if (GS) {
```
